# DinoBektesevic/lfd

Measured on AMD Instinct MI355X. Metric: SDSS frames/sec (2048x1489) full detecttrails pipe, higher is better.
Workload: dtype f32

## Files before the change

lfd_amd/csrc/k_hough.h:

```cpp
#pragma once
#include "common.h"
#include "../../include/lfdmi.h"

#define PIXLIST_WORDS 8
#define CHUNK_MAX 64
__device__ __forceinline__ uint32_t chunk_entry(int y, int x0, int len) {
    return ((uint32_t)(len - 1) << 26) | ((uint32_t)y << 13) | (uint32_t)x0;
}

__global__ void __launch_bounds__(256)
k_pixlist(const u64 *bits0, const u64 *bits1, uint32_t *list0, uint32_t *list1, int *counters, int cm_a, int cm_b, int h, int w,
          size_t list_cap, int *accum_clear, int acc_n, size_t acc_stride, const int *active, int need_detect) {
    int g = blockIdx.y, im = blockIdx.z;
    const u64 *bits = im ? bits1 : bits0;
    uint32_t *list = im ? list1 : list0;
    const int cidx = im ? C_NPIX_BOX : C_NPIX_EQU, cidx_b = im ? C_NPIXB_BOX : C_NPIXB_EQU, nnz_idx = im ? C_NNZ_BOX : C_NNZ_EQU;
    if (accum_clear) accum_clear += (size_t)im * acc_stride;
    if (slot_off(active, counters, g)) return;
    int *cnt = counters + g * C_COUNT;
    if (need_detect && !cnt[C_DETECT]) return;
    int wq = LFD_WQ(w);
    if (accum_clear)
        for (int k = blockIdx.x * 256 + threadIdx.x; k < acc_n; k += gridDim.x * 256) accum_clear[(size_t)g * 2 * acc_stride + k] = 0;
    const int nw = h * wq;
// ... 328 lines not shown
            u64 v = pg[k];
            if (v < prev && v > best) best = v;
        }
        for (int off = 32; off > 0; off >>= 1) {
            u64 o = __shfl_down(best, off);
            if (o > best) best = o;
        }
        if (lfd_lane() == 0) red[threadIdx.x >> 6] = best;
        __syncthreads();
        if (threadIdx.x == 0) {
            u64 b = red[0];
            for (int k = 1; k < 4; k++) if (red[k] > b) b = red[k];
            prev_s = b;
            float ro = 0.f, th = 0.f;
            if (b) key_to_line(b, numrho, rho, theta, &ro, &th);
            lg[2 * round] = ro;
            lg[2 * round + 1] = th;
        }
        __syncthreads();
        prev = prev_s;
        if (!prev) {
            if (threadIdx.x == 0)
                for (int r2 = round + 1; r2 < K; r2++) { lg[2 * r2] = 0.f; lg[2 * r2 + 1] = 0.f; }
            break;
        }
    }
}

__global__ void __launch_bounds__(1024)
k_hough_sort(u64 *peaks, const int *counters, float *lines, int max_lines, int numrho, float rho,
             float theta, size_t peak_cap) {
    int g = blockIdx.y, im = blockIdx.x;
    const int *cnt = counters + g * C_COUNT;
    if (cnt[C_OVERFLOW]) return;
    u64 *pg = peaks + ((size_t)g * 2 + im) * peak_cap;
    int n = cnt[im ? C_NPEAK_BOX : C_NPEAK_EQU];
    if ((size_t)n > peak_cap) n = (int)peak_cap;
    int np2 = 1;
    while (np2 < n) np2 <<= 1;
    for (int k = n + threadIdx.x; k < np2; k += 1024) pg[k] = 0;
    __syncthreads();
    for (int size = 2; size <= np2; size <<= 1)
        for (int stride = size >> 1; stride > 0; stride >>= 1) {
            for (int t = threadIdx.x; t < (np2 >> 1); t += 1024) {
                int lo = 2 * t - (t & (stride - 1));
                int hi = lo + stride;
                bool desc = ((lo & size) == 0);
                u64 a = pg[lo], b = pg[hi];
                if (desc ? (a < b) : (a > b)) { pg[lo] = b; pg[hi] = a; }
            }
            __syncthreads();
        }
    int m = min(n, max_lines);
    float *lg = lines + (size_t)g * max_lines * 2;
    for (int k = threadIdx.x; k < m; k += 1024) key_to_line(pg[k], numrho, rho, theta, &lg[2 * k], &lg[2 * k + 1]);
}

__device__ double np_pairwise_dev(const double *a, int n) {
    if (n < 8) {
        double res = 0.;
        for (int i = 0; i < n; i++) res = __dadd_rn(res, a[i]);
        return res;
    }
    double r[8], res;
    int i;
    for (int j = 0; j < 8; j++) r[j] = a[j];
    for (i = 8; i < n - (n % 8); i += 8)
        for (int j = 0; j < 8; j++) r[j] = __dadd_rn(r[j], a[i + j]);
    res = __dadd_rn(__dadd_rn(__dadd_rn(r[0], r[1]), __dadd_rn(r[2], r[3])),
                    __dadd_rn(__dadd_rn(r[4], r[5]), __dadd_rn(r[6], r[7])));
    for (; i < n; i++) res = __dadd_rn(res, a[i]);
    return res;
}
__device__ double np_mean_dev(const double *a, int n) {
    return __ddiv_rn(__dadd_rn(a[0], np_pairwise_dev(a + 1, n - 1)), (double)n);
}

struct TailParams {
    int navg;
    double dro, thetaTresh, lineSetTresh;
    int which;
};

__global__ void k_finalize(const float *lines, const int *counters, lfdmi_result *res, int *need_dim,
                           int *pass_flags, const int *active, TailParams tp, int G) {
    int g = blockIdx.x * blockDim.x + threadIdx.x;
    if (g >= G) return;
    if (active && !active[g]) { if (need_dim) need_dim[g] = 0; return; }
    const int *cnt = counters + g * C_COUNT;
    lfdmi_result r = res[g];
    r.detection = cnt[C_DETECT];
    r.rejected_by_theta = 0;
    r.n_lines_equ = r.n_lines_box = 0;
    if (cnt[C_OVERFLOW]) {
        r.status = LFDMI_ERR_CAPACITY;
        r.x1 = max(cnt[C_NRUNF], cnt[C_NRUNB]);
        r.y1 = cnt[C_NKEYS];
        r.x2 = cnt[C_NSLOTS];
        r.y2 = max(max(cnt[C_NPIX_EQU], cnt[C_NPIX_BOX]), max(cnt[C_NPIXB_EQU], cnt[C_NPIXB_BOX]));
        r.n_lines_equ = max(cnt[C_NPEAK_EQU], cnt[C_NPEAK_BOX]);
    }
    if (r.detection && r.status == 0) {
        int n1 = cnt[C_NPEAK_EQU], n2 = cnt[C_NPEAK_BOX];
        r.n_lines_equ = n1; r.n_lines_box = n2;
        if (n1 == 0 || n2 == 0) {
            r.status = LFDMI_ERR_NOLINES;
        } else {
            int K = tp.navg;
            const float *l1 = lines + ((size_t)g * 2 + 0) * K * 2, *l2 = lines + ((size_t)g * 2 + 1) * K * 2;
            double ro1[LFDMI_MAX_SET_LINES], ro2[LFDMI_MAX_SET_LINES], t1[LFDMI_MAX_SET_LINES],
                t2[LFDMI_MAX_SET_LINES];
            for (int i = 0; i < K; i++) {
                ro1[i] = ro2[i] = t1[i] = t2[i] = 0.;
                if (i >= n1) continue;
                ro1[i] = l1[2 * i];
                if (i >= n2) continue;
                ro2[i] = l2[2 * i];
                t1[i] = l1[2 * i + 1];
                t2[i] = l2[2 * i + 1];
            }
            bool rej = fabs(__dsub_rn(np_mean_dev(ro1, K), np_mean_dev(ro2, K))) > tp.dro;
            if (!rej) {
                double mx = t1[0], mn = t1[0];
                for (int i = 1; i < K; i++) { mx = fmax(mx, t1[i]); mn = fmin(mn, t1[i]); }
                rej = fabs(__dsub_rn(mx, mn)) > tp.thetaTresh;
            }
            if (!rej) {
                double mx = t2[0], mn = t2[0];
                for (int i = 1; i < K; i++) { mx = fmax(mx, t2[i]); mn = fmin(mn, t2[i]); }
                rej = fabs(__dsub_rn(mx, mn)) > tp.thetaTresh;
            }
            if (!rej) {
                for (int i = 0; i < K; i++) ro1[i] = fabs(__dsub_rn(t1[i], t2[i]));
                rej = np_mean_dev(ro1, K) > tp.lineSetTresh;
            }
            if (rej) r.rejected_by_theta = 1;
            else { r.found = tp.which; r.rho = l1[0]; r.theta = l1[1]; }
        }
    }
    res[g] = r;
    pass_flags[g] |= (tp.which == 1) ? (r.detection ? 1 : 0) : (2 | (r.detection ? 4 : 0));
    if (need_dim) need_dim[g] = (r.found == 0 && r.status == 0) ? 1 : 0;
}

__global__ void k_hough_reset(int *counters, int G) {
    int g = blockIdx.x * blockDim.x + threadIdx.x;
    if (g >= G) return;
    int *cnt = counters + g * C_COUNT;
    cnt[C_NPIX_EQU] = 0; cnt[C_NPIX_BOX] = 0; cnt[C_NPIXB_EQU] = 0; cnt[C_NPIXB_BOX] = 0; cnt[C_NPEAK_EQU] = 0; cnt[C_NPEAK_BOX] = 0;
    cnt[C_NNZ_EQU] = 0; cnt[C_NNZ_BOX] = 0;
}

__global__ void k_init_results(lfdmi_result *res, int *pass_flags, int G) {
    int g = blockIdx.x * blockDim.x + threadIdx.x;
    if (g >= G) return;
    pass_flags[g] = 0;
    lfdmi_result r;
    r.status = 0; r.found = 0; r.rho = 0.f; r.theta = 0.f;
    r.x1 = r.y1 = r.x2 = r.y2 = 0;
    r.n_lines_equ = r.n_lines_box = 0; r.detection = 0; r.rejected_by_theta = 0;
    res[g] = r;
}
```

lfd_amd/csrc/k_image.h:

```cpp
#pragma once
#include <type_traits>
#include "common.h"
#include "../../include/lfdmi.h"

struct RsDev {
    int defaultxy, maxxy, magcount, filter_index;
    double pixscale, maxmagdiff, filter_cap;
};

__device__ __forceinline__ void py_slice(long start, long stop, long len, int *a, int *b) {
    if (start < 0) { start += len; if (start < 0) start = 0; } else if (start > len) start = len;
    if (stop < 0) { stop += len; if (stop < 0) stop = 0; } else if (stop > len) stop = len;
    *a = (int)start; *b = (int)stop;
}

__global__ void __launch_bounds__(256)
k_rs_boxes(int h, int w, int max_obj, const int *count, const float *rowc, const float *colc, const float *psfmag,
           const float *petro90, const int *nobserve, const int *ndetect, RsDev p, int4 *boxes) {
    const int f = blockIdx.y, i = blockIdx.x * 256 + threadIdx.x;
    if (i >= max_obj) return;
    int r0 = 0, r1 = 0, c0 = 0, c1 = 0;
    if (i < count[f]) {
        size_t o5 = ((size_t)f * max_obj + i) * 5, o1 = (size_t)f * max_obj + i;
        int fi = p.filter_index;
        long x = (long)ceil((double)colc[o5 + fi]);
        long y = (long)ceil((double)rowc[o5 + fi]);
        long mags[5];
        for (int k = 0; k < 5; k++) mags[k] = (long)ceil((double)psfmag[o5 + k]);
        bool ok = (double)mags[fi] < p.filter_cap;
        int cnt = 0;
        for (int j = 0; j < 5; j++)
            for (int k = j + 1; k < 5; k++) {
                long d = mags[j] - mags[k];
                if (d < 0) d = -d;
                if ((double)d > p.maxmagdiff) cnt++;
            }
        ok = ok && (p.magcount >= cnt);
        long dxy = p.defaultxy;
        long pet = (long)ceil((double)petro90[o5 + fi]);
        if (pet > 0) dxy = (long)((double)pet / p.pixscale) + 10;
        if (dxy > p.maxxy) dxy = p.defaultxy;
        ok = ok && (nobserve[o1] == ndetect[o1]);
        if (ok) {
            py_slice(x - dxy, x + dxy, h, &r0, &r1);
            py_slice(y - dxy, y + dxy, w, &c0, &c1);
        }
    }
    boxes[(size_t)f * max_obj + i] = make_int4(r0, r1, c0, c1);
}

__global__ void __launch_bounds__(256)
k_rs_fill(float *frames, int h, int w, int max_obj, const int *count, const int4 *boxes, int bx0) {
    int f = blockIdx.y, i = (blockIdx.x + bx0) * 4 + (threadIdx.x >> 6), lane = threadIdx.x & 63;
    if (i >= max_obj) return;
    const int4 bx = boxes[(size_t)f * max_obj + i];
    const int r0 = __builtin_amdgcn_readfirstlane(bx.x), r1 = __builtin_amdgcn_readfirstlane(bx.y);
    const int c0 = __builtin_amdgcn_readfirstlane(bx.z), c1 = __builtin_amdgcn_readfirstlane(bx.w);
    int nc = c1 - c0;
    if (r1 <= r0 || nc <= 0) return;
    float *img = frames + (size_t)f * h * w;
    if (nc <= 32) {
        for (int r = r0 + (lane >> 5); r < r1; r += 2)
            if ((lane & 31) < nc) img[(size_t)r * w + c0 + (lane & 31)] = 0.0f;
    } else {
        for (int r = r0; r < r1; r++)
            for (int c = c0 + lane; c < c1; c += 64) img[(size_t)r * w + c] = 0.0f;
    }
}

#define RS_SORT_MIN 1024
#define RS_SORT_MAXH 8192
__global__ void __launch_bounds__(1024)
k_rs_sort(int h, int max_obj, const int *count, const int4 *boxes, int4 *sboxes, int *rowstart) {
    const int f = blockIdx.x, n = min(count[f], max_obj);
    __shared__ int cur[RS_SORT_MAXH + 1];
    __shared__ int wsum[16];
    const int4 *bx = boxes + (size_t)f * max_obj;
    for (int r = threadIdx.x; r <= h; r += 1024) cur[r] = 0;
    __syncthreads();
    for (int i = threadIdx.x; i < n; i += 1024) {
        const int4 b = bx[i];
        if (b.y > b.x && b.w > b.z) atomicAdd(&cur[b.x], 1);
    }
    __syncthreads();
    const int per = (h + 1 + 1023) / 1024, r0 = threadIdx.x * per, lane = threadIdx.x & 63, wv = threadIdx.x >> 6;
    int loc = 0;
    for (int k = 0; k < per; k++) if (r0 + k <= h) loc += cur[r0 + k];
    int inc = loc;
    for (int off = 1; off < 64; off <<= 1) { int t = __shfl_up(inc, off); if (lane >= off) inc += t; }
    if (lane == 63) wsum[wv] = inc;
    __syncthreads();
    int base = inc - loc;
    for (int k = 0; k < wv; k++) base += wsum[k];
    for (int k = 0; k < per; k++)
        if (r0 + k <= h) {
            const int c = cur[r0 + k];
            cur[r0 + k] = base;
            rowstart[(size_t)f * (h + 1) + r0 + k] = base;
            base += c;
        }
    __syncthreads();
    for (int i = threadIdx.x; i < n; i += 1024) {
// ... 486 lines not shown
    }
    const uint8_t *gs = gsrc + (size_t)g * N;
    const u64 *db = dbits + (size_t)g * nw;
    __shared__ unsigned short qlist[4][512];
    __shared__ int qyq[4][64];
    const int wvi = threadIdx.x >> 6;
    qyq[wvi][lane] = (y << 8) | q;
    u64 rem = e;
    for (;;) {
        const int cnt = min(__popcll(rem), 8);
        int incl = cnt;
        for (int off = 1; off < 64; off <<= 1) {
            int t = __shfl_up(incl, off);
            if (lane >= off) incl += t;
        }
        const int total = __shfl(incl, 63);
        if (total == 0) break;
        int o = incl - cnt;
        for (int k = 0; k < cnt; k++) {
            const int bb = __ffsll((long long)rem) - 1;
            rem &= rem - 1;
            qlist[wvi][o++] = (unsigned short)((lane << 6) | bb);
        }
        __builtin_amdgcn_wave_barrier();
        for (int t = lane; t < total; t += 64) {
            const unsigned ent = qlist[wvi][t];
            const int yq = qyq[wvi][ent >> 6];
            const int yy0 = yq >> 8, x = ((yq & 0xff) << 6) + (int)(ent & 63u);
            auto val = [&](int yy, int xx) -> unsigned {
                if (yy < 0 || yy >= h || xx < 0 || xx >= w) return 255u;
                return (unsigned)gs[(size_t)yy * w + xx] + (unsigned)((db[(size_t)yy * wq + (xx >> 6)] >> (xx & 63)) & 1ull);
            };
            unsigned m = 255u;
            if (kh == 3 && kw == 3 && x >= 1 && x + 2 < w && yy0 >= 1 && yy0 + 1 < h) {
                unsigned gv[3];
                u64 bw0[3], bw1[3];
                const int xb = x - 1, wi = xb >> 6, sh = xb & 63;
#pragma unroll
                for (int k = 0; k < 3; k++) {
                    const size_t ro = (size_t)(yy0 + k - 1);
                    uint32_t t4;
                    __builtin_memcpy(&t4, gs + ro * w + xb, 4);
                    gv[k] = t4;
                    bw0[k] = db[ro * wq + wi];
                    bw1[k] = sh > 61 ? db[ro * wq + wi + 1] : 0ull;
                }
#pragma unroll
                for (int k = 0; k < 3; k++) {
                    const unsigned bits = (unsigned)((bw0[k] >> sh) | (sh > 61 ? bw1[k] << (64 - sh) : 0ull)) & 7u;
                    m = min(m, (gv[k] & 0xffu) + (bits & 1u));
                    m = min(m, ((gv[k] >> 8) & 0xffu) + ((bits >> 1) & 1u));
                    m = min(m, ((gv[k] >> 16) & 0xffu) + ((bits >> 2) & 1u));
                }
            } else if (kh == 3 && kw == 3) {
                unsigned v9[9];
#pragma unroll
                for (int k = 0; k < 9; k++) v9[k] = val(yy0 + k / 3 - 1, x + k % 3 - 1);
#pragma unroll
                for (int k = 0; k < 9; k++) m = min(m, v9[k]);
            } else {
                for (int dy = 0; dy < kh; dy++)
                    for (int dx = 0; dx < kw; dx++) m = min(m, val(yy0 + dy - ay, x + dx - ax));
            }
            d[(size_t)yy0 * w + x] = (uint8_t)m;
        }
        __builtin_amdgcn_wave_barrier();
    }
    }
}

__global__ void __launch_bounds__(256)
k_hist_u8(const uint8_t *src, size_t N, int *hist) {
    int g = blockIdx.y;
    __shared__ int sh[256];
    sh[threadIdx.x] = 0;
    __syncthreads();
    const uint8_t *s = src + (size_t)g * N;
    for (size_t k = (size_t)blockIdx.x * 256 + threadIdx.x; k < N; k += (size_t)gridDim.x * 256)
        atomicAdd(&sh[s[k]], 1);
    __syncthreads();
    if (sh[threadIdx.x]) atomicAdd(&hist[g * 256 + threadIdx.x], sh[threadIdx.x]);
}

__global__ void __launch_bounds__(256)
k_lut(const int *hist, int total, uint8_t *lut, const int *active) {
    int g = blockIdx.x, t = threadIdx.x;
    if (active && !active[g]) return;
    __shared__ int cum[256];
    __shared__ int first;
    int hv = hist[g * 256 + t];
    cum[t] = hv;
    if (t == 0) first = 256;
    __syncthreads();
    if (hv) atomicMin(&first, t);
    for (int off = 1; off < 256; off <<= 1) {
        int v = (t >= off) ? cum[t - off] : 0;
        __syncthreads();
        cum[t] += v;
        __syncthreads();
    }
    int f = first;
    if (f >= 256) { lut[g * 256 + t] = 0; return; }
    int hf = hist[g * 256 + f];
    unsigned out;
    if (hf == total) out = (unsigned)f;
    else if (t <= f) out = 0;
    else {
        float scale = __fdiv_rn(255.f, (float)(total - hf));
        out = sat_u8_f32(__fmul_rn((float)(cum[t] - cum[f]), scale));
    }
    lut[g * 256 + t] = (uint8_t)out;
}

__global__ void __launch_bounds__(256)
k_apply_lut(const uint8_t *src, const uint8_t *lut, uint8_t *dst, size_t N) {
    int g = blockIdx.y;
    __shared__ uint8_t l[256];
    l[threadIdx.x] = lut[g * 256 + threadIdx.x];
    __syncthreads();
    for (size_t k = (size_t)blockIdx.x * 256 + threadIdx.x; k < N; k += (size_t)gridDim.x * 256)
        dst[(size_t)g * N + k] = l[src[(size_t)g * N + k]];
}

typedef unsigned short dcw_us2 __attribute__((ext_vector_type(2)));
__device__ __forceinline__ uint32_t dcw_pkmax(uint32_t a, uint32_t b) {
    return __builtin_bit_cast(uint32_t, __builtin_elementwise_max(__builtin_bit_cast(dcw_us2, a), __builtin_bit_cast(dcw_us2, b)));
}
__device__ __forceinline__ uint32_t dcw_pkmin(uint32_t a, uint32_t b) {
    return __builtin_bit_cast(uint32_t, __builtin_elementwise_min(__builtin_bit_cast(dcw_us2, a), __builtin_bit_cast(dcw_us2, b)));
}
template <int S, int NWT, bool MIN = false>
__device__ __forceinline__ void dcw_shift_max(uint32_t (&E)[NWT], uint32_t (&O)[NWT], int nw) {
    constexpr int K = S / 4, R = S % 4;
#pragma unroll
    for (int i = 0; i < NWT; i++) {
        if (i >= nw || i + K + 1 >= NWT) continue;
        uint32_t e2, o2;
        if constexpr (R == 0) { e2 = E[i + K]; o2 = O[i + K]; }
        else if constexpr (R == 1) { e2 = O[i + K]; o2 = __builtin_amdgcn_alignbyte(E[i + K + 1], E[i + K], 2); }
        else if constexpr (R == 2) { e2 = __builtin_amdgcn_alignbyte(E[i + K + 1], E[i + K], 2); o2 = __builtin_amdgcn_alignbyte(O[i + K + 1], O[i + K], 2); }
        else { e2 = __builtin_amdgcn_alignbyte(O[i + K + 1], O[i + K], 2); o2 = E[i + K + 1]; }
        E[i] = MIN ? dcw_pkmin(E[i], e2) : dcw_pkmax(E[i], e2);
        O[i] = MIN ? dcw_pkmin(O[i], o2) : dcw_pkmax(O[i], o2);
    }
}
template <int KW, bool MIN = false, int BASE = 12>
__device__ __forceinline__ uint32_t dcw_hmax(const uint32_t *rw, int jj) {
    constexpr int AX = KW / 2, R0 = (BASE - AX) & 3, Q0 = (BASE - AX) >> 2;
    constexpr int NB = KW + 3, NW = (NB + 3) / 4, NR = (R0 + NB + 3) / 4, NWT = NW + 9;
    uint32_t raw[NR + 1];
#pragma unroll
    for (int i = 0; i < NR; i++) raw[i] = rw[Q0 + jj + i];
    raw[NR] = 0;
    uint32_t E[NWT], O[NWT];
#pragma unroll
    for (int i = 0; i < NWT; i++) {
        uint32_t a = 0;
        if (i < NW) a = R0 ? __builtin_amdgcn_alignbyte(raw[i + 1 <= NR ? i + 1 : NR], raw[i], R0) : raw[i];
        E[i] = a & 0x00FF00FFu;
        O[i] = (a >> 8) & 0x00FF00FFu;
    }
    constexpr int P = KW >= 16 ? 16 : (KW >= 8 ? 8 : (KW >= 4 ? 4 : (KW >= 2 ? 2 : 1))), D = KW - P;
    constexpr int need1 = 4 + D + (P > 8 ? 8 : 0) + (P > 4 ? 4 : 0) + (P > 2 ? 2 : 0);
    if constexpr (P >= 2) dcw_shift_max<1, NWT, MIN>(E, O, (need1 + 3) / 4);
    constexpr int need2 = need1 - 2;
    if constexpr (P >= 4) dcw_shift_max<2, NWT, MIN>(E, O, (need2 + 3) / 4);
    constexpr int need4 = need2 - 4;
    if constexpr (P >= 8) dcw_shift_max<4, NWT, MIN>(E, O, (need4 + 3) / 4);
    if constexpr (P >= 16) dcw_shift_max<8, NWT, MIN>(E, O, (4 + D + 3) / 4);
    if constexpr (D > 0) dcw_shift_max<D, NWT, MIN>(E, O, 1);
    return E[0] | (O[0] << 8);
}

#define MORPH_TW 64
#define MORPH_TH 32

template <int OP>
__global__ void __launch_bounds__(256)
k_morph_rect(const uint8_t *src, uint8_t *dst, u64 *bits, const uint8_t *lut, int h, int w, int kh,
             int kw, const int *active) {
    int g = blockIdx.z;
    if (active && !active[g]) return;
    extern __shared__ uint8_t sm[];
    const int IH = MORPH_TH + kh - 1, IW = MORPH_TW + kw - 1;
    uint8_t *tin = sm;
    uint8_t *tmp = sm + ((IH * IW + 15) & ~15);
    __shared__ uint8_t slut[256];
    const int fill = OP ? 255 : 0;
    int x0 = blockIdx.x * MORPH_TW, y0 = blockIdx.y * MORPH_TH;
    int ay = kh / 2, ax = kw / 2;
    size_t N = (size_t)h * w;
    const uint8_t *s = src + (size_t)g * N;
    if (lut) slut[threadIdx.x] = lut[g * 256 + threadIdx.x];
    for (int idx = threadIdx.x; idx < IH * IW; idx += 256) {
// ... 1095 lines not shown
```

lfd_amd/csrc/lfdmi.hip:

```cpp
#include <hip/hip_runtime.h>

#include <math.h>
#include <stdio.h>
#include <stdlib.h>
#include <time.h>
#include <pthread.h>
#include <sched.h>
#include <string.h>

#include <atomic>
#include <condition_variable>
#include <string>
#include <thread>
#include <mutex>
#include <memory>
#include <vector>

#include "../../include/lfdmi.h"
#include "common.h"
#include "k_ccl.h"
#include "k_hough.h"
#include "k_image.h"
#include "k_rect.h"
#include "k_frame.h"
// ... 20 lines not shown
struct TimedSpan { hipEvent_t a, b; int group, pass, det; };

struct CallChunk {
    int c0, nc;
    bool general_on, scan_fused;
    long long growths;
};
struct PendingCall {
    int kind = 0;
    int status = 0;
    bool finished = false;
    void *frames = nullptr;
    size_t frame_bytes = 0;
    int dtype = 0, n = 0, h = 0, w = 0, loc = 0;
    bool host_blot = false;
    lfdmi_catalog cat{};
    bool has_cat = false, has_rs = false;
    lfdmi_rs_params rs{};
    lfdmi_params p1{}, p2{};
    std::vector<uint8_t> kern;
    int flip = 0, dim = 0, prep_mode = 0, n_scales = 1;
    double rhos[LFDMI_MAX_SCALES] = {0};
    lfdmi_result *results = nullptr;
    std::vector<CallChunk> chunks;
    void *pin = nullptr;
    size_t pin_bytes = 0;
    int *flags_h = nullptr;
    lfdmi_result *rec_h = nullptr;
    int4 *boxes_h = nullptr;
    hipEvent_t done = nullptr;
};

struct lfdmi_ctx {
    int device = 0, H = 0, W = 0, G = 0, wq = 0;
    size_t N = 0;
    hipStream_t stream = nullptr;
    bool own_stream = true;
    hipStream_t side[2] = {nullptr, nullptr};
    hipEvent_t ev_fork = nullptr, ev_join[2] = {nullptr, nullptr};
    std::string err;
    uint8_t *gray = nullptr, *tmp = nullptr, *equ = nullptr, *lut = nullptr, *mask = nullptr;
    int *hist = nullptr;
    u64 *candb = nullptr, *strongb = nullptr, *edgeb = nullptr, *equb = nullptr, *boxb = nullptr;
    int *Lf = nullptr, *YMf = nullptr, *FLf = nullptr, *Lb = nullptr, *YMb = nullptr, *FLb = nullptr;
    int *SBf = nullptr, *SBb = nullptr, *PAb = nullptr, *ROWf = nullptr, *ROWb = nullptr;
    int *scanf_ = nullptr, *scanb_ = nullptr;
    int run_cap = 0;
    int4 *keys = nullptr;
    int *bigkeys = nullptr, *medkeys = nullptr;
    int *wl_fg = nullptr, *wl_bg = nullptr;
    int2 *rowext = nullptr;
    int *quads = nullptr;
    uint32_t *pix_equ = nullptr, *pix_box = nullptr;
    int *accum = nullptr;
    u64 *peaks = nullptr;
    float *lines = nullptr, *tab = nullptr;
    int *counters = nullptr, *need_dim = nullptr;
    uint8_t *zero_block = nullptr;
    size_t zero_bytes = 0, zero_counters_off = 0;
    uint8_t *zero_block2 = nullptr;
    size_t zero_bytes2 = 0;
    u64 *cellbm2 = nullptr;
    u64 *candmask = nullptr;
    u64 *fullbits = nullptr;
    int *hist2 = nullptr;
    bool fuse_dual = false;
    u64 *dbits = nullptr, *nzd = nullptr;
    bool sparse_erode_fill = true;
    bool delta_dim = true;
    int delta_state = 0;
    int dual_state = 0;
    int2 *rsa = nullptr;
    long long *prof = nullptr;
    u64 *cellbm = nullptr;
    int bm_bands = 0;
    bool use_cellbm = true;
    int4 *segcnt = nullptr;
    int *fg_keys = nullptr;
    bool fg_keys_on = true;
    int *fb_fg = nullptr, *fb_bg = nullptr;
    int *perm = nullptr;
    const int *perm_cur = nullptr;
    bool use_perm = true;
    int *perm_tiles = nullptr;
    bool use_tile_perm = true;
    bool sky_fast = true;
    bool vote_classes = true;
    bool rs_fold_on = true;
    bool rs_fold = false;
    const int *rs_count_dev = nullptr; int rs_max_obj = 0;
    int rs_fill_at = 13;
    int rs_fill_at0 = 3, rs_fill_part = 0;
    float *rs_fill_frames = nullptr;
    int rs_fill_nc = 0, rs_fill_h = 0, rs_fill_w = 0;
    hipEvent_t ev_rsfill = nullptr;
    bool rs_fill_inflight = false;
    bool scan_fused = true;
    u64 *scan_partial = nullptr;
    int scan_epoch = 0;
    int scan_spin = 4096;
    bool rects_prep = true;
    bool vote_balance = true;
    lfdmi_result *res_dev = nullptr;
    void *res_host = nullptr;
    bool worst = false;
    lfdmi_ctx *spill = nullptr;
    long long n_spilled = 0;
    long long n_scan_giveups = 0, n_general_reruns = 0, n_general_chunks = 0, n_chunks = 0, n_cap_growths = 0;
    bool grow_on = true;
    bool scan_fused_cfg = true;
    int scan_quiet = 0, scan_rearm = 64;
    size_t bytes = 0;
    double min_rho = 1.0;
    void *scratch = nullptr;
    size_t scratch_bytes = 0;
    int last_h = 0, last_w = 0;
    int quiet_chunks = 0;
    void *feed_pin[2] = {nullptr, nullptr}, *feed_dev[2] = {nullptr, nullptr};
    size_t feed_bytes = 0, feed_pin_bytes = 0;
    bool feed_cpus_known = false;
    hipStream_t feed_copy = nullptr, feed_copy2 = nullptr;
    hipEvent_t feed_mid = nullptr;
    int feed_streams = 2;
    hipEvent_t feed_up[2] = {nullptr, nullptr};
    int feed_threads = 4;
    size_t feed_chunk_bytes = 800u << 20;
    std::vector<int> feed_cpus;
    int fail_chunk = -1;
    int4 *rs_sboxes = nullptr;
    int *rs_rowstart = nullptr;
    size_t rs_rowstart_cap = 0;
    bool rs_sorted = false;
    int rs_sort_min = RS_SORT_MIN;
    int rs_hmax = 0;
    int4 *rs_boxes = nullptr;
    size_t rs_boxes_cap = 0;
    void *stage = nullptr;
    size_t stage_bytes = 0;
    void *cat_dev = nullptr;
    size_t cat_bytes = 0;
    int key_cap = 0, slot_cap = 0;
    size_t acc_cap = 0, peak_cap = 0, list_cap = 0, peak_worst = 0;
    struct HoughTab {
        double rho = -1, theta = -1;
        int h = 0, w = 0, numangle = 0, numrho = 0;
        long long stamp = 0;
        std::vector<float> host;
    } tabs[LFDMI_MAX_SCALES];
    long long tab_clock = 0;
    int tab_cur = 0;
    int numangle = 0, numrho = 0;
    bool timing = false;
    uint64_t timing_mask = 0;
    std::vector<TimedSpan> spans;
    std::vector<hipEvent_t> ev_pool;
    float t_ms[TG_COUNT] = {0};
    int t_n[TG_COUNT] = {0};
    long long t_units[TG_COUNT] = {0};
    int stage_mode = -1;
    bool stages_valid = false;
    bool eroded_valid = false;
    int vote_split = 4;
    int vote_aw = -1;
    int pe_rows = 12;
    bool fuse_prep_erode = true;
    bool general_seen = false, general_on = true;
// ... 118 lines not shown
static void worst_caps(int h, int w, lfdmi_caps *c) {
    size_t N = (size_t)h * w;
    c->run_cap = (int)((size_t)h * (w / 2 + 1) + 16);
    c->key_cap = (int)(N / 2 + 16);
    c->slot_cap = (int)(2 * N + 4 * (size_t)h + 16);
    c->list_cap = (int)N;
    c->peak_cap = 0;
    c->min_rho = 1.0;
}

extern "C" void lfdmi_default_caps(int max_h, int max_w, lfdmi_caps *out) {
    size_t N = (size_t)max_h * max_w;
    lfdmi_caps wc;
    worst_caps(max_h, max_w, &wc);
    auto pick = [](size_t want, size_t floor_, int worst) { size_t v = want > floor_ ? want : floor_; return (int)(v < (size_t)worst ? v : (size_t)worst); };
    out->run_cap = pick(N / 16, 16384, wc.run_cap);
    out->key_cap = pick(N / 256, 4096, wc.key_cap);
    out->slot_cap = pick(N / 16, 16384, wc.slot_cap);
    out->list_cap = pick(N / 16, 16384, wc.list_cap);
    out->peak_cap = 65536;
    out->min_rho = 5.0;
}

static int create_impl(int device, int max_h, int max_w, int max_inflight, const lfdmi_caps *caps_in, lfdmi_ctx **out) {
    if (!out || max_h <= 0 || max_w <= 0 || max_inflight <= 0 || max_h > 8191 || max_w > 8191) return LFDMI_ERR_ARG;
    lfdmi_ctx *ctx = new lfdmi_ctx();
    *out = ctx;
    ctx->device = device; ctx->H = max_h; ctx->W = max_w; ctx->G = max_inflight;
    if (const char *e = getenv("LFDMI_FRAME_CCL")) ctx->frame_ccl = atoi(e) != 0;
    if (const char *e = getenv("LFDMI_FUSE_PREP_ERODE")) ctx->fuse_prep_erode = atoi(e) != 0;
    if (const char *e = getenv("LFDMI_FUSE_DUAL")) ctx->fuse_dual = atoi(e) != 0;
    if (const char *e = getenv("LFDMI_DELTA_DIM")) ctx->delta_dim = atoi(e) != 0;
    if (const char *e = getenv("LFDMI_SPARSE_ERODE_FILL")) ctx->sparse_erode_fill = atoi(e) != 0;
    if (const char *e = getenv("LFDMI_VOTE_SPLIT")) { int v = atoi(e); if (v >= 1 && v <= 16) ctx->vote_split = v; }
    if (const char *e = getenv("LFDMI_VOTE_AW")) { int v = atoi(e); if (*e && v >= 0 && v <= 6) ctx->vote_aw = v; }
    if (const char *e = getenv("LFDMI_PE_ROWS")) { int v = atoi(e); if (v >= 2 && v <= 64) ctx->pe_rows = v; }
    if (const char *e = getenv("LFDMI_FRAME_DBG")) ctx->frame_dbg = atoi(e);
    if (const char *e = getenv("LFDMI_FRAME_RUNCAP")) { int v = atoi(e); if (v >= 0 && v < FRAME_RUNCAP) ctx->frame_runcap = v; }
    if (const char *e = getenv("LFDMI_FRAME_LDS")) {
        int v = atoi(e);
        if (v >= 32 && v <= FRAME_RUNCAP) { ctx->frame_lds = (v + 31) & ~31; ctx->frame_runcap = std::min(ctx->frame_runcap, ctx->frame_lds); }
    }
    if (const char *e = getenv("LFDMI_DC_SUBSTRIPS")) { int v = atoi(e); if (v >= 1 && v <= 64) ctx->dc_substrips = v; }
    if (const char *e = getenv("LFDMI_DC_STRIP")) { int v = atoi(e); if (v >= 1 && v <= DCW_MAXS) ctx->dc_strip = v; }
    if (const char *e = getenv("LFDMI_DC_TILELIST")) ctx->dc_tilelist = atoi(e) != 0;
    if (const char *e = getenv("LFDMI_DC_PARTS")) { int v = atoi(e); if (v >= 1 && v <= 4096) ctx->dc_parts = v; }
    if (const char *e = getenv("LFDMI_FEED_STREAMS")) { int v = atoi(e); if (v == 1 || v == 2) ctx->feed_streams = v; }
    if (const char *e = getenv("LFDMI_FEED_THREADS")) { int v = atoi(e); if (v >= 1 && v <= 64) ctx->feed_threads = v; }
    if (const char *e = getenv("LFDMI_FEED_MB")) { int v = atoi(e); if (v >= 0 && v <= 8192) ctx->feed_chunk_bytes = (size_t)v << 20; }
    ctx->N = (size_t)max_h * max_w;
    ctx->wq = LFD_WQ(max_w);
    size_t N = ctx->N, G = (size_t)max_inflight, BW = (size_t)max_h * ctx->wq;
    lfdmi_caps wc, caps;
    worst_caps(max_h, max_w, &wc);
    if (caps_in) caps = *caps_in; else lfdmi_default_caps(max_h, max_w, &caps);
    if (const char *e = getenv("LFDMI_WORST_CASE")) if (atoi(e)) caps = wc;
    auto cap = [](int v, int worst) { return (v <= 0 || v > worst) ? worst : v; };
    ctx->run_cap = cap(caps.run_cap, wc.run_cap);
    ctx->key_cap = cap(caps.key_cap, wc.key_cap);
    ctx->slot_cap = cap(caps.slot_cap, wc.slot_cap);
    ctx->list_cap = (size_t)cap(caps.list_cap, wc.list_cap);
    ctx->min_rho = caps.min_rho >= 1.0 ? caps.min_rho : 1.0;
    int na, nr;
    lfdmi_hough_dims(max_h, max_w, ctx->min_rho, LFD_PI / 180, &na, &nr);
    ctx->acc_cap = (size_t)(na + 2) * (nr + 2);
    size_t peak_worst = next_pow2((size_t)na * nr);
    ctx->peak_cap = caps.peak_cap > 0 ? next_pow2((size_t)caps.peak_cap) : peak_worst;
    if (ctx->peak_cap > peak_worst) ctx->peak_cap = peak_worst;
    ctx->peak_worst = peak_worst;
    ctx->worst = ctx->run_cap == wc.run_cap && ctx->key_cap == wc.key_cap && ctx->slot_cap == wc.slot_cap &&
                 ctx->list_cap == (size_t)wc.list_cap && ctx->peak_cap == peak_worst && ctx->min_rho <= 1.0;
    HIPCHK(hipSetDevice(device));
    HIPCHK(hipStreamCreateWithFlags(&ctx->stream, hipStreamNonBlocking));
    for (int i = 0; i < 2; i++) {
        HIPCHK(hipStreamCreateWithFlags(&ctx->side[i], hipStreamNonBlocking));
        HIPCHK(hipEventCreateWithFlags(&ctx->ev_join[i], hipEventDisableTiming));
    }
    HIPCHK(hipEventCreateWithFlags(&ctx->ev_fork, hipEventDisableTiming));
    HIPCHK(hipEventCreateWithFlags(&ctx->ev_rsfill, hipEventDisableTiming));
    RET(dmalloc(ctx, &ctx->gray, G * N));
    RET(dmalloc(ctx, &ctx->tmp, G * N));
    RET(dmalloc(ctx, &ctx->equ, G * N));
    RET(dmalloc(ctx, &ctx->lut, G * 256));
    RET(dmalloc(ctx, &ctx->mask, (size_t)LFDMI_MAX_MORPH_K * LFDMI_MAX_MORPH_K * 2));
    RET(dmalloc(ctx, &ctx->candb, G * BW));
    RET(dmalloc(ctx, &ctx->strongb, G * BW));
    RET(dmalloc(ctx, &ctx->edgeb, G * BW));
    RET(dmalloc(ctx, &ctx->equb, G * BW));
    RET(dmalloc(ctx, &ctx->boxb, G * BW));
    RET(dmalloc(ctx, &ctx->dbits, G * BW));
    RET(dmalloc(ctx, &ctx->nzd, G * BW));
    for (int **p : {&ctx->Lf, &ctx->YMf, &ctx->FLf, &ctx->Lb, &ctx->YMb, &ctx->FLb, &ctx->SBf, &ctx->SBb, &ctx->PAb,
                    &ctx->ROWf, &ctx->ROWb})
        RET(dmalloc(ctx, p, G * ctx->run_cap));
    if (const char *e = getenv("LFDMI_DC_PROFILE")) ctx->dc_profile = atoi(e) != 0;
    if (const char *e = getenv("LFDMI_DC_SPECIALIZE")) ctx->dc_specialize = atoi(e) != 0;
    if (getenv("LFDMI_FRAME_PROFILE") || ctx->dc_profile) RET(dmalloc(ctx, &ctx->prof, G * 16));
    RET(dmalloc(ctx, &ctx->rsa, G * FRAME_RUNCAP));
    ctx->bm_bands = (max_h + CELLBM_ROWS - 1) / CELLBM_ROWS;
    if (const char *e = getenv("LFDMI_CELLBM")) ctx->use_cellbm = atoi(e) != 0;
    ctx->tile_cap = ((max_h + DCW_TH - 1) / DCW_TH) * ((max_w + CANNY_TW - 1) / CANNY_TW);
    RET(dmalloc(ctx, &ctx->tile_list, G * ctx->tile_cap));
    RET(dmalloc(ctx, &ctx->segcnt, G * SCAN_MAX_SEG));
    RET(dmalloc(ctx, &ctx->perm, G));
    RET(dmalloc(ctx, &ctx->perm_tiles, G));
    if (const char *e = getenv("LFDMI_TILE_PERM")) ctx->use_tile_perm = atoi(e) != 0;
    if (const char *e = getenv("LFDMI_SKY_FAST")) ctx->sky_fast = atoi(e) != 0;
    if (const char *e = getenv("LFDMI_VOTE_CLASSES")) ctx->vote_classes = atoi(e) != 0;
    if (const char *e = getenv("LFDMI_VOTE_BALANCE")) ctx->vote_balance = atoi(e) != 0;
    if (const char *e = getenv("LFDMI_RECTS_PREP")) ctx->rects_prep = atoi(e) != 0;
    if (const char *e = getenv("LFDMI_RS_FOLD")) ctx->rs_fold_on = atoi(e) != 0;
    if (const char *e = getenv("LFDMI_RS_SORT_MIN")) ctx->rs_sort_min = atoi(e);
    if (const char *e = getenv("LFDMI_SCAN_FUSED")) ctx->scan_fused = atoi(e) != 0;
    ctx->scan_fused_cfg = ctx->scan_fused;
    if (const char *e = getenv("LFDMI_GROW")) ctx->grow_on = atoi(e) != 0;
    if (const char *e = getenv("LFDMI_SCAN_REARM")) ctx->scan_rearm = std::max(1, atoi(e));
    if (const char *e = getenv("LFDMI_SCAN_SPIN")) ctx->scan_spin = std::max(0, atoi(e));
    if (const char *e = getenv("LFDMI_SCAN_EPOCH0")) ctx->scan_epoch = atoi(e) & ((1 << 22) - 1);
    if (const char *e = getenv("LFDMI_RS_FILL_AT")) ctx->rs_fill_at = atoi(e);
    if (const char *e = getenv("LFDMI_RS_FILL_AT0")) ctx->rs_fill_at0 = atoi(e);
    if (const char *e = getenv("LFDMI_PERM")) ctx->use_perm = atoi(e) != 0;
    RET(dmalloc(ctx, &ctx->fb_fg, G));
    RET(dmalloc(ctx, &ctx->fg_keys, G));
    HIPCHK(hipMemsetAsync(ctx->fg_keys, 0, G * sizeof(int), ctx->stream));
    if (const char *e = getenv("LFDMI_FG_KEYS")) ctx->fg_keys_on = atoi(e) != 0;
    RET(dmalloc(ctx, &ctx->fb_bg, G));
    RET(dmalloc(ctx, &ctx->scanf_, G * BW));
    RET(dmalloc(ctx, &ctx->scanb_, G * BW));
    RET(dmalloc(ctx, &ctx->keys, G * ctx->key_cap));
    RET(dmalloc(ctx, &ctx->bigkeys, G * ctx->key_cap));
    RET(dmalloc(ctx, &ctx->medkeys, G * ctx->key_cap));
    RET(dmalloc(ctx, &ctx->wl_fg, G * BW));
    RET(dmalloc(ctx, &ctx->wl_bg, G * BW));
    RET(dmalloc(ctx, &ctx->rowext, G * ctx->slot_cap));
    RET(dmalloc(ctx, &ctx->quads, G * ctx->key_cap * 8));
    RET(dmalloc(ctx, &ctx->pix_equ, G * 2 * ctx->list_cap));
    RET(dmalloc(ctx, &ctx->pix_box, G * 2 * ctx->list_cap));
    RET(dmalloc(ctx, &ctx->accum, G * 2 * ctx->acc_cap));
    RET(dmalloc(ctx, &ctx->peaks, G * 2 * ctx->peak_cap));
    RET(dmalloc(ctx, &ctx->lines, G * 2 * LFDMI_MAX_SET_LINES * 2));
    RET(dmalloc(ctx, &ctx->tab, (size_t)LFDMI_MAX_SCALES * 2 * MAX_ANGLES));
    {
        size_t nb_cnt = G * C_COUNT * sizeof(int), nb_hist = G * 256 * sizeof(int), nb_bm = G * ctx->bm_bands * CELLBM_WORDS * sizeof(u64);
        uint8_t *blk = nullptr;
        RET(dmalloc(ctx, &blk, nb_bm + nb_hist + nb_cnt));
        ctx->cellbm = (u64 *)blk;
        ctx->hist = (int *)(blk + nb_bm);
        ctx->counters = (int *)(blk + nb_bm + nb_hist);
        ctx->zero_block = blk;
        ctx->zero_bytes = nb_bm + nb_hist + nb_cnt;
        ctx->zero_counters_off = nb_bm + nb_hist;
        uint8_t *blk2 = nullptr;
        RET(dmalloc(ctx, &blk2, nb_bm + nb_hist));
        ctx->cellbm2 = (u64 *)blk2;
        ctx->hist2 = (int *)(blk2 + nb_bm);
        ctx->zero_block2 = blk2;
        ctx->zero_bytes2 = nb_bm + nb_hist;
        RET(dmalloc(ctx, &ctx->fullbits, G * (size_t)max_h * ((max_w + 255) >> 8)));
        RET(dmalloc(ctx, &ctx->candmask, G * (size_t)((max_h + MORPH_TH - 1) / MORPH_TH) * 2));
    }
    RET(dmalloc(ctx, &ctx->need_dim, G));
    RET(dmalloc(ctx, &ctx->scan_partial, G * SCAN_MAX_BLK));
    HIPCHK(hipMemsetAsync(ctx->scan_partial, 0, G * SCAN_MAX_BLK * sizeof(u64), ctx->stream));
    {
        char *blk = nullptr;
        RET(dmalloc(ctx, &blk, G * sizeof(int) + G * LFDMI_MAX_SCALES * sizeof(lfdmi_result)));
        ctx->pass_flags = (int *)blk;
        ctx->res_dev = (lfdmi_result *)(blk + G * sizeof(int));
        HIPCHK(hipHostMalloc(&ctx->res_host, G * sizeof(int) + G * sizeof(lfdmi_result), hipHostMallocDefault));
    }
    HIPCHK(hipFuncSetAttribute((const void *)k_hough_vote<6>, hipFuncAttributeMaxDynamicSharedMemorySize, 160 * 1024 - 64));
    HIPCHK(hipFuncSetAttribute((const void *)k_hough_vote<5>, hipFuncAttributeMaxDynamicSharedMemorySize, 160 * 1024 - 64));
    HIPCHK(hipFuncSetAttribute((const void *)k_hough_vote<4>, hipFuncAttributeMaxDynamicSharedMemorySize, 160 * 1024 - 64));
    HIPCHK(hipFuncSetAttribute((const void *)k_hough_vote<3>, hipFuncAttributeMaxDynamicSharedMemorySize, 160 * 1024 - 64));
    HIPCHK(hipFuncSetAttribute((const void *)k_hough_vote<2>, hipFuncAttributeMaxDynamicSharedMemorySize, 160 * 1024 - 64));
    HIPCHK(hipFuncSetAttribute((const void *)k_hough_vote<1>, hipFuncAttributeMaxDynamicSharedMemorySize, 160 * 1024 - 64));
    HIPCHK(hipFuncSetAttribute((const void *)k_hough_vote<0>, hipFuncAttributeMaxDynamicSharedMemorySize, 160 * 1024 - 64));
    HIPCHK(hipFuncSetAttribute((const void *)k_rects_big, hipFuncAttributeMaxDynamicSharedMemorySize, 160 * 1024 - 64));
    HIPCHK(hipFuncSetAttribute((const void *)k_dilate_canny_v, hipFuncAttributeMaxDynamicSharedMemorySize, 64 * 1024));
    HIPCHK(hipFuncSetAttribute((const void *)k_frame_fg, hipFuncAttributeMaxDynamicSharedMemorySize, 160 * 1024 - 1024));
    HIPCHK(hipFuncSetAttribute((const void *)k_prep_erode<false, 0>, hipFuncAttributeMaxDynamicSharedMemorySize, 140 * 1024));
    HIPCHK(hipFuncSetAttribute((const void *)k_prep_erode<false, 1>, hipFuncAttributeMaxDynamicSharedMemorySize, 140 * 1024));
    HIPCHK(hipFuncSetAttribute((const void *)k_prep_erode<false, 2>, hipFuncAttributeMaxDynamicSharedMemorySize, 140 * 1024));
    HIPCHK(hipFuncSetAttribute((const void *)k_prep_erode<false, 3>, hipFuncAttributeMaxDynamicSharedMemorySize, 140 * 1024));
    HIPCHK(hipFuncSetAttribute((const void *)k_prep_erode<true, LFDMI_PREP_BRIGHT_THEN_DIM>, hipFuncAttributeMaxDynamicSharedMemorySize, 140 * 1024));
    HIPCHK(hipFuncSetAttribute((const void *)k_frame_contours, hipFuncAttributeMaxDynamicSharedMemorySize,
                               (FRAME_RUNCAP + 4 * (FRAME_RUNCAP / 32)) * (int)sizeof(int)));
    HIPCHK(hipFuncSetAttribute((const void *)k_morph_rect<0>, hipFuncAttributeMaxDynamicSharedMemorySize, 64 * 1024));
    HIPCHK(hipFuncSetAttribute((const void *)k_morph_rect<1>, hipFuncAttributeMaxDynamicSharedMemorySize, 64 * 1024));
    return 0;
}

extern "C" int lfdmi_ctx_create(int device, int max_h, int max_w, int max_inflight, lfdmi_ctx **out) {
    return create_impl(device, max_h, max_w, max_inflight, nullptr, out);
}
extern "C" int lfdmi_ctx_create_sized(int device, int max_h, int max_w, int max_inflight, const lfdmi_caps *caps, lfdmi_ctx **out) {
    return create_impl(device, max_h, max_w, max_inflight, caps, out);
}
extern "C" int64_t lfdmi_ctx_bytes(lfdmi_ctx *ctx) {
    return ctx ? (int64_t)(ctx->bytes + ctx->trail.bytes + (ctx->spill ? ctx->spill->bytes : 0)) : 0;
}
extern "C" int64_t lfdmi_spill_count(lfdmi_ctx *ctx) { return ctx ? ctx->n_spilled : 0; }
extern "C" int lfdmi_get_stats(lfdmi_ctx *ctx, int64_t *out, int n) {
    if (!ctx || !out || n < 0 || n > LFDMI_STAT_COUNT) return LFDMI_ERR_ARG;
// ... 254 lines not shown
    }
    return 0;
}

static int rs_fill_point(lfdmi_ctx *ctx, int k) {
    if (!ctx->rs_fill_frames) return 0;
    const bool first = k >= 0 && k == ctx->rs_fill_at0 && ctx->rs_fill_part == 0 && !ctx->rs_sorted;
    const bool rest = k < 0 || k == ctx->rs_fill_at;
    if (!first && !rest) return 0;
    float *fr = ctx->rs_fill_frames;
    static const int side_i = getenv("LFDMI_RS_FILL_SIDE") ? (atoi(getenv("LFDMI_RS_FILL_SIDE")) & 1) : 1;
    hipStream_t sd = ctx->side[side_i];
    HIPCHK(hipEventRecord(ctx->ev_rsfill, ctx->stream));
    HIPCHK(hipStreamWaitEvent(sd, ctx->ev_rsfill, 0));
    {
        Span sp(ctx, KID_REMOVESTARS, 0, sd);
        if (ctx->rs_sorted)
            k_rs_fill_bands<<<dim3((ctx->rs_fill_h + RS_BAND_ROWS - 1) / RS_BAND_ROWS, ctx->rs_fill_nc), 256, 0, sd>>>(
                fr, ctx->rs_fill_h, ctx->rs_fill_w, ctx->rs_max_obj, ctx->rs_sboxes, ctx->rs_rowstart, ctx->rs_hmax);
        else {
            static const double frac = getenv("LFDMI_RS_FILL_FRAC") ? atof(getenv("LFDMI_RS_FILL_FRAC")) : 0.5;
            const int nblk = (ctx->rs_max_obj + 3) / 4, half = std::max(0, std::min(nblk, (int)(nblk * frac)));
            const int b0 = ctx->rs_fill_part ? half : 0, b1 = first ? half : nblk;
            if (b1 > b0)
                k_rs_fill<<<dim3(b1 - b0, ctx->rs_fill_nc), 256, 0, sd>>>(fr, ctx->rs_fill_h, ctx->rs_fill_w, ctx->rs_max_obj,
                                                                          ctx->rs_count_dev, ctx->rs_boxes, b0);
        }
        KCHK("k_rs_fill");
    }
    HIPCHK(hipEventRecord(ctx->ev_rsfill, sd));
    ctx->rs_fill_inflight = true;
    if (first) ctx->rs_fill_part = 1;
    else { ctx->rs_fill_frames = nullptr; ctx->rs_fill_part = 0; }
    return 0;
}

static dim3 word_grid(int h, int w, int n) { return dim3((unsigned)((h * LFD_WQ(w) + 255) / 256), (unsigned)n); }

static int run_prep(lfdmi_ctx *ctx, const void *src, int dtype, int nc, int h, int w, int flip, int mode,
                    double minFlux, double addFlux, const int *active, bool zeroed = false, u64 *fullbits = nullptr,
                    const lfdmi_params *delta_dim = nullptr) {
    if (!zeroed) {
        HIPCHK(hipMemsetAsync(ctx->hist, 0, (size_t)nc * 256 * sizeof(int), ctx->stream));
        HIPCHK(hipMemsetAsync(ctx->cellbm, 0, (size_t)nc * ctx->bm_bands * CELLBM_WORDS * sizeof(u64), ctx->stream));
    }
    {
        Span sp(ctx, KID_PREP_HIST);
        static const int prep_rows = [] {
            const char *e = getenv("LFDMI_PREP_ROWS");
            int v = e ? atoi(e) : 8;
            return (v == 1 || v == 2 || v == 4 || v == 8 || v == 16) ? v : 8;
        }();
        const dim3 pgrid((h + prep_rows - 1) / prep_rows, nc);
#define LFD_PREP_LAUNCH(M_)                                                                                                          \
    k_prep_hist<M_><<<pgrid, 256, 0, ctx->stream>>>(src, dtype, h, w, flip, mode, minFlux, addFlux, ctx->gray, ctx->hist, ctx->cellbm, \
                                                    ctx->bm_bands, active, fullbits, prep_rows)
        if (delta_dim) {
#define LFD_PREP_DELTA(P_, RS_)                                                                                                       \
    k_prep_hist<1, true, P_, RS_><<<pgrid, 256, 0, ctx->stream>>>(src, dtype, h, w, flip, mode, minFlux, addFlux, ctx->gray, ctx->hist, \
                                                              ctx->cellbm, ctx->bm_bands, active, fullbits, prep_rows, ctx->dbits,    \
                                                              ctx->hist2, (float)delta_dim->minFlux, (float)delta_dim->addFlux, ctx->nzd, sky_fast, \
                                                              ctx->rs_sorted ? ctx->rs_sboxes : ctx->rs_boxes, ctx->rs_count_dev, ctx->rs_max_obj, \
                                                              ctx->rs_sorted ? ctx->rs_rowstart : nullptr, ctx->rs_hmax)
            const bool sky_on = ctx->sky_fast;
            const float mfa = (float)delta_dim->minFlux + (float)delta_dim->addFlux;
            const int sky_fast = (sky_on && mode == LFDMI_PREP_BRIGHT && mfa > 0.5f) ? 1 : 0;
            const bool rs = ctx->rs_fold && w <= RS_MAXW && prep_rows <= RS_MAXROWS;
            if ((float)delta_dim->minFlux > 0.f) { if (rs) LFD_PREP_DELTA(true, true); else LFD_PREP_DELTA(true, false); }
            else { if (rs) LFD_PREP_DELTA(false, true); else LFD_PREP_DELTA(false, false); }
#undef LFD_PREP_DELTA
        } else
        if (dtype == LFDMI_F32 && (w & 3) == 0) {
            switch (mode & 3) {
            case 0: LFD_PREP_LAUNCH(0); break;
            case 1: LFD_PREP_LAUNCH(1); break;
            case 2: LFD_PREP_LAUNCH(2); break;
            default: LFD_PREP_LAUNCH(3); break;
            }
        } else LFD_PREP_LAUNCH(-1);
#undef LFD_PREP_LAUNCH
        KCHK("k_prep_hist");
    }
    Span sp(ctx, KID_LUT);
    k_lut<<<nc, 256, 0, ctx->stream>>>(ctx->hist, h * w, ctx->lut, active);
    KCHK("k_lut");
    return 0;
}

static bool all_ones(const uint8_t *k, int kh, int kw) {
    for (int i = 0; i < kh * kw; i++) if (!k[i]) return false;
    return true;
}

static int run_morph(lfdmi_ctx *ctx, const uint8_t *src, uint8_t *dst, u64 *bits, const uint8_t *lut, const uint8_t *kernel,
                     int kh, int kw, int op, int nc, int h, int w, const int *active, const u64 *fullbits = nullptr, u64 *cellout = nullptr,
                     bool *marked = nullptr, bool sparse_fill = false) {
    if (marked) *marked = false;
    if (!kernel || kh <= 0 || kw <= 0 || kh > LFDMI_MAX_MORPH_K || kw > LFDMI_MAX_MORPH_K)
        return fail(ctx, LFDMI_ERR_UNSUPPORTED, "structuring element must be 1..31 on both sides");
    Span sp(ctx, op ? KID_ERODE : KID_DILATE);
    if (all_ones(kernel, kh, kw) && (w % 16) == 0) {
        int IH = MORPH_TH + kh - 1;
        size_t lds = (size_t)IH * (MORPH_TW + 2 * MORPH_HALO) + (size_t)IH * MORPH_TW * 2 + (size_t)MORPH_TH * MORPH_TW;
        dim3 grid((w + MORPH_TW - 1) / MORPH_TW, (h + MORPH_TH - 1) / MORPH_TH, nc);
        const u64 *cand = nullptr;
        if (op == 1 && fullbits && kw >= 7 && !lut && !bits && grid.x <= 128 && kh <= 33) {
            sparse_fill = sparse_fill && cellout && kh <= 9 && kw <= 33;
            k_erode_cand<<<dim3(grid.y, nc), 64, 0, ctx->stream>>>(fullbits, ctx->candmask, dst, h, w, kh, active, sparse_fill ? 0 : 1);
            KCHK("k_erode_cand");
            cand = ctx->candmask;
        }
        if (op == 0) k_morph_rect_v<0><<<grid, 256, lds, ctx->stream>>>(src, dst, bits, lut, h, w, kh, kw, active, cellout, ctx->bm_bands);
        else if (cand) {
            dim3 rgrid(grid.y, nc);
            if (kh == 9 && kw == 9 && ctx->dc_specialize)
                k_morph_rect_rows<1, 9, 9><<<rgrid, 256, lds, ctx->stream>>>(src, dst, lut, h, w, kh, kw, active, cand, cellout, ctx->bm_bands);
            else k_morph_rect_rows<1><<<rgrid, 256, lds, ctx->stream>>>(src, dst, lut, h, w, kh, kw, active, cand, cellout, ctx->bm_bands);
        } else if (kh == 9 && kw == 9 && ctx->dc_specialize)
            k_morph_rect_v<1, 9, 9><<<grid, 256, lds, ctx->stream>>>(src, dst, bits, lut, h, w, kh, kw, active, cellout, ctx->bm_bands);
        else k_morph_rect_v<1><<<grid, 256, lds, ctx->stream>>>(src, dst, bits, lut, h, w, kh, kw, active, cellout, ctx->bm_bands);
        if (marked) *marked = cellout != nullptr;
        KCHK("k_morph_rect_v");
        if (cand && sparse_fill) {
            k_fill_around<<<dim3(grid.y, nc), 64, 0, ctx->stream>>>(cand, cellout, ctx->bm_bands, dst, h, w, active);
            KCHK("k_fill_around");
        }
    } else if (all_ones(kernel, kh, kw)) {
        int IH = MORPH_TH + kh - 1, IW = MORPH_TW + kw - 1;
        size_t lds = ((size_t)(IH * IW + 15) & ~(size_t)15) + (size_t)IH * MORPH_TW;
        dim3 grid((w + MORPH_TW - 1) / MORPH_TW, (h + MORPH_TH - 1) / MORPH_TH, nc);
        if (op == 0) k_morph_rect<0><<<grid, 256, lds, ctx->stream>>>(src, dst, bits, lut, h, w, kh, kw, active);
        else k_morph_rect<1><<<grid, 256, lds, ctx->stream>>>(src, dst, bits, lut, h, w, kh, kw, active);
        KCHK("k_morph_rect");
    } else {
        uint8_t *m = ctx->mask + (op ? LFDMI_MAX_MORPH_K * LFDMI_MAX_MORPH_K : 0);
        HIPCHK(hipMemcpyAsync(m, kernel, (size_t)kh * kw, hipMemcpyHostToDevice, ctx->stream));
        dim3 grid((w + 63) / 64, (h + 3) / 4, nc);
        if (op == 0) k_morph_generic<0><<<grid, 256, 0, ctx->stream>>>(src, dst, bits, lut, m, h, w, kh, kw, active);
        else k_morph_generic<1><<<grid, 256, 0, ctx->stream>>>(src, dst, bits, lut, m, h, w, kh, kw, active);
        KCHK("k_morph_generic");
    }
    return 0;
}

static int run_scan(lfdmi_ctx *ctx, const u64 *bits, int val, int *scan, int cidx, int nc, int h, int w, int *wl_fg, int *wl_bg,
                    u64 *clear, const int *active) {
    int nseg = (h * LFD_WQ(w) + 63) / 64;
    dim3 grid((nseg + SCANW_WAVES * SCAN_SEGS - 1) / (SCANW_WAVES * SCAN_SEGS), nc);
    if (ctx->scan_fused && (int)grid.x <= SCAN_MAX_BLK) {
        if (++ctx->scan_epoch >= (1 << 22)) {
            HIPCHK(hipMemsetAsync(ctx->scan_partial, 0, (size_t)ctx->G * SCAN_MAX_BLK * sizeof(u64), ctx->stream));
            ctx->scan_epoch = 1;
        }
        k_scan_fused<<<grid, 64 * SCANW_WAVES, 0, ctx->stream>>>(bits, val, ctx->scan_partial, ctx->scan_epoch, ctx->scan_spin, ctx->pass_flags, scan, h, w, wl_fg, wl_bg, clear,
                                                                  ctx->counters, cidx, ctx->run_cap, active);
        KCHK("k_scan_fused");
        return 0;
    }
    k_scan_count<<<grid, 64 * SCANW_WAVES, 0, ctx->stream>>>(bits, val, ctx->segcnt, h, w, wl_fg != nullptr, active);
    KCHK("k_scan_count");
    k_scan_bases<<<nc, SCAN_THREADS, 0, ctx->stream>>>(ctx->segcnt, ctx->counters, cidx, h, w, ctx->run_cap, wl_fg != nullptr, active);
    KCHK("k_scan_bases");
    k_scan_write<<<grid, 64 * SCANW_WAVES, 0, ctx->stream>>>(bits, val, ctx->segcnt, scan, h, w, wl_fg, wl_bg, clear, active);
    KCHK("k_scan_write");
    return 0;
}
// ... 421 lines not shown
                                                                   ctx->acc_cap, active, need_detect, rng, balance); \
        break;
        switch (aw_log2) {
            LFD_LAUNCH_VOTE(6) LFD_LAUNCH_VOTE(5) LFD_LAUNCH_VOTE(4) LFD_LAUNCH_VOTE(3) LFD_LAUNCH_VOTE(2)
            LFD_LAUNCH_VOTE(1) LFD_LAUNCH_VOTE(0)
        }
#undef LFD_LAUNCH_VOTE
        KCHK("k_hough_vote");
    }
    { Span sp(ctx, KID_PEAKS, need_detect);
    static const int peak_rows = getenv("LFDMI_PEAK_ROWS") ? std::max(8, atoi(getenv("LFDMI_PEAK_ROWS"))) : 32;
    k_hough_peaks<<<dim3(std::min(32, std::max(1, nr / peak_rows)), n_img, nc), std::min(256, (na + 63) / 64 * 64), 0, ctx->stream>>>(ctx->accum, ctx->peaks, ctx->counters, na, nr, threshold,
                                                                ctx->acc_cap, ctx->peak_cap, active, need_detect);
    KCHK("k_hough_peaks"); }
    if (K > 0) {
        Span sp(ctx, KID_TOPK, need_detect);
        k_hough_topk<<<dim3(n_img, nc), 256, 0, ctx->stream>>>(ctx->peaks, ctx->counters, ctx->lines, K, nr, (float)rho, (float)theta,
                                                               ctx->peak_cap, active, need_detect);
        KCHK("k_hough_topk");
    }
    return 0;
}

static int check_params(lfdmi_ctx *ctx, const lfdmi_params *p, bool dim) {
    if (!p) return fail(ctx, LFDMI_ERR_ARG, "params NULL");
    if (p->gaussKernel < 0 || p->gaussKernel > 31 || (p->gaussKernel > 0 && (p->gaussKernel & 1) == 0))
        return fail(ctx, LFDMI_ERR_ARG, "gaussKernel must be 0 (off) or odd, 1..31");
    if (p->nlinesInSet < 1 || p->nlinesInSet > LFDMI_MAX_SET_LINES) return fail(ctx, LFDMI_ERR_ARG, "nlinesInSet out of range");
    if (!p->dilateKernel) return fail(ctx, LFDMI_ERR_ARG, "dilateKernel NULL");
    if (dim && !p->erodeKernel) return fail(ctx, LFDMI_ERR_ARG, "erodeKernel NULL");
    return 0;
}

static int prep_erode_rows(const lfdmi_ctx *ctx, int w, int kh) {
    int BR = ctx->pe_rows;
    while (BR > 2 && (size_t)(2 * BR + kh - 1) * (w + 32) > 60 * 1024) BR >>= 1;
    if ((size_t)(2 * BR + kh - 1) * (w + 32) + 16 > 140 * 1024) return 0;
    return BR >= 2 * (kh - 1) ? BR : 0;
}

static bool can_fuse_prep_erode(const lfdmi_ctx *ctx, int dtype, int w, const uint8_t *kernel, int kh, int kw) {
    if (!ctx->fuse_prep_erode || ctx->keep_equ || dtype != LFDMI_F32 || (w % 16) != 0) return false;
    if (!kernel || kh <= 0 || kw <= 0 || kh > LFDMI_MAX_MORPH_K || kw > LFDMI_MAX_MORPH_K || !all_ones(kernel, kh, kw)) return false;
    return kw / 2 <= 16 && kw - 1 - kw / 2 <= 16 && prep_erode_rows(ctx, w, kh) > 0;
}

static int run_prep_erode(lfdmi_ctx *ctx, const void *src, int nc, int h, int w, int flip, int mode, double minFlux, double addFlux,
                          int kh, int kw, const int *active, bool from_bits = false) {
    int BR = prep_erode_rows(ctx, w, kh);
    size_t lds = (size_t)(2 * BR + kh - 1) * (w + 32) + 16;
    if (from_bits) {
        Span sp(ctx, KID_BITS_ERODE);
        const int nwords = h * LFD_WQ(w);
        k_bits_erode<<<dim3((nwords + 256 * BE_REP - 1) / (256 * BE_REP), nc), 256, 0, ctx->stream>>>(ctx->gray, ctx->dbits, ctx->nzd, ctx->tmp, ctx->cellbm2,
                                                                             ctx->bm_bands, h, w, kh, kw, active);
        KCHK("k_bits_erode");
        return 0;
    }
    {
        Span sp(ctx, KID_PREP_ERODE);
#define LFD_PE_LAUNCH(M_)                                                                                                             \
    k_prep_erode<false, M_><<<dim3((h + BR - 1) / BR, nc), PE_THREADS, lds, ctx->stream>>>(                                           \
        (const float *)src, h, w, flip, mode, (float)minFlux, (float)addFlux, ctx->tmp, ctx->hist, kh, kw, BR, ctx->cellbm, ctx->bm_bands, \
        active, nullptr, nullptr, nullptr)
        switch (mode & 3) {
        case 0: LFD_PE_LAUNCH(0); break;
        case 1: LFD_PE_LAUNCH(1); break;
        case 2: LFD_PE_LAUNCH(2); break;
        default: LFD_PE_LAUNCH(3); break;
        }
#undef LFD_PE_LAUNCH
        KCHK("k_prep_erode");
    }
    Span sp(ctx, KID_LUT);
    k_lut<<<nc, 256, 0, ctx->stream>>>(ctx->hist, h * w, ctx->lut, active);
    KCHK("k_lut");
    return 0;
}

static int run_prep_dual(lfdmi_ctx *ctx, const void *src, int nc, int h, int w, int flip, const lfdmi_params *dimp) {
    int kh = dimp->erode_kh, kw = dimp->erode_kw;
    int BR = prep_erode_rows(ctx, w, kh);
    size_t lds = (size_t)(2 * BR + kh - 1) * (w + 32) + 16;
    HIPCHK(hipMemsetAsync(ctx->zero_block2, 0, ctx->zero_bytes2, ctx->stream));
    {
        Span sp(ctx, KID_PREP_DUAL);
        k_prep_erode<true, LFDMI_PREP_BRIGHT_THEN_DIM><<<dim3((h + BR - 1) / BR, nc), PE_THREADS, lds, ctx->stream>>>((const float *)src, h, w, flip, LFDMI_PREP_BRIGHT_THEN_DIM,
                                                                              (float)dimp->minFlux, (float)dimp->addFlux, ctx->tmp, ctx->hist2, kh, kw, BR,
                                                                              ctx->cellbm2, ctx->bm_bands, nullptr, ctx->gray, ctx->hist, ctx->cellbm);
        KCHK("k_prep_dual");
    }
    Span sp(ctx, KID_LUT);
    k_lut<<<nc, 256, 0, ctx->stream>>>(ctx->hist, h * w, ctx->lut, nullptr);
    KCHK("k_lut");
    return 0;
}

static int run_front(lfdmi_ctx *ctx, const void *src, int dtype, int nc, int h, int w, int flip, int prep_mode, bool dim,
                     const lfdmi_params *p, const int *active, const lfdmi_params *dual_dim = nullptr) {
    const uint8_t *dil_src = ctx->gray;
    const u64 *bm = ctx->cellbm;
    ctx->eroded_valid = dim;
    ctx->perm_cur = nullptr;
    if (active && ctx->use_perm) {
        k_active_perm<<<1, 64, 0, ctx->stream>>>(active, nc, ctx->perm);
        KCHK("k_active_perm");
        ctx->perm_cur = ctx->perm;
    }
    if (dim && ctx->delta_state == 2) {
        HIPCHK(hipMemsetAsync(ctx->zero_block + ctx->zero_counters_off, 0, ctx->zero_bytes - ctx->zero_counters_off, ctx->stream));
        HIPCHK(hipMemsetAsync(ctx->cellbm2, 0, (size_t)nc * ctx->bm_bands * CELLBM_WORDS * sizeof(u64), ctx->stream));
        { Span sp(ctx, KID_LUT);
          k_lut<<<nc, 256, 0, ctx->stream>>>(ctx->hist2, h * w, ctx->lut, active);
          KCHK("k_lut"); }
        RET(run_prep_erode(ctx, nullptr, nc, h, w, 0, 0, 0, 0, p->erode_kh, p->erode_kw, active, true));
        dil_src = ctx->tmp;
        bm = ctx->cellbm2;
    } else
    if (dim && ctx->dual_state == 2) {
        HIPCHK(hipMemsetAsync(ctx->zero_block + ctx->zero_counters_off, 0, ctx->zero_bytes - ctx->zero_counters_off, ctx->stream));
        Span sp(ctx, KID_LUT);
        k_lut<<<nc, 256, 0, ctx->stream>>>(ctx->hist2, h * w, ctx->lut, active);
        KCHK("k_lut");
        dil_src = ctx->tmp;
        bm = ctx->cellbm2;
    } else {
    HIPCHK(hipMemsetAsync(ctx->zero_block, 0, ctx->zero_bytes, ctx->stream));
    if (!dim && dual_dim && ctx->delta_state != 1) {
        RET(run_prep_dual(ctx, src, nc, h, w, flip, dual_dim));
    } else
    if (dim && can_fuse_prep_erode(ctx, dtype, w, p->erodeKernel, p->erode_kh, p->erode_kw)) {
        RET(run_prep_erode(ctx, src, nc, h, w, flip, prep_mode, p->minFlux, p->addFlux, p->erode_kh, p->erode_kw, active));
        dil_src = ctx->tmp;
    } else {
        const bool wide = dim && p->erode_kw >= 7 && dtype == LFDMI_F32 && (w & 3) == 0 && p->erode_kh <= 33;
        if (dim) HIPCHK(hipMemsetAsync(ctx->zero_block2, 0, ctx->zero_bytes2, ctx->stream));
        const lfdmi_params *dd = (!dim && ctx->delta_state == 1) ? dual_dim : nullptr;
        if (dd) HIPCHK(hipMemsetAsync(ctx->hist2, 0, (size_t)nc * 256 * sizeof(int), ctx->stream));
        RET(run_prep(ctx, src, dtype, nc, h, w, flip, prep_mode, p->minFlux, p->addFlux, active, true, wide ? ctx->fullbits : nullptr, dd));
        RET(rs_fill_point(ctx, 1));
        if (dim) {
            bool marked = false;
            const bool only_tiles = wide && !ctx->keep_equ && ctx->sparse_erode_fill && p->gaussKernel <= 0 && ctx->use_cellbm && ctx->dc_tilelist &&
                                    p->dilate_kh <= 9 && p->dilate_kh <= DCW_MAXKH && can_fuse_dilate_canny(p->dilateKernel, p->dilate_kh, p->dilate_kw, w) &&
                                    (w + CANNY_TW - 1) / CANNY_TW <= 128 && (h + DCW_TH - 1) / DCW_TH <= DCT_MAXBANDS;
            RET(run_morph(ctx, ctx->gray, ctx->tmp, nullptr, nullptr, p->erodeKernel, p->erode_kh, p->erode_kw, 1, nc, h, w, active,
                          wide ? ctx->fullbits : nullptr, ctx->cellbm2, &marked, only_tiles));
            if (only_tiles) ctx->eroded_valid = false;
            dil_src = ctx->tmp;
            if (marked) bm = ctx->cellbm2;
        }
    }
    }
    if (p->gaussKernel > 0) {
        RET(run_morph(ctx, dil_src, ctx->equ, ctx->equb, ctx->lut, p->dilateKernel, p->dilate_kh, p->dilate_kw, 0, nc, h, w, active));
        RET(ensure_scratch(ctx, (size_t)ctx->G * ctx->N));
        RET(run_gauss(ctx, ctx->equ, (uint8_t *)ctx->scratch, nc, h, w, p->gaussKernel, p->gaussSigma, active));
        RET(run_canny(ctx, (const uint8_t *)ctx->scratch, nc, h, w, 0, 255, active, false, true));
    } else if (can_fuse_dilate_canny(p->dilateKernel, p->dilate_kh, p->dilate_kw, w)) {
        RET(run_dilate_canny(ctx, dil_src, nc, h, w, ctx->lut, p->dilate_kh, p->dilate_kw, active, ctx->use_cellbm ? bm : nullptr));
        RET(rs_fill_point(ctx, 2 + 10 * ctx->cur_pass));
        RET(run_canny(ctx, ctx->equ, nc, h, w, 0, 255, active, true, true));
    } else {
        RET(run_morph(ctx, dil_src, ctx->equ, ctx->equb, ctx->lut, p->dilateKernel, p->dilate_kh, p->dilate_kw, 0, nc, h, w, active));
        RET(run_canny(ctx, ctx->equ, nc, h, w, 0, 255, active, false, true));
    }
    return run_rects(ctx, nc, h, w, p->contoursMode, p->contoursMethod, p->minAreaRectMinLen, p->lwTresh, active);
}

static int run_tail(lfdmi_ctx *ctx, int nc, int h, int w, double rho, bool dim, const lfdmi_params *p, const int *active,
                    int *need_dim, lfdmi_result *res, bool again) {
    if (again) {
        k_hough_reset<<<(nc + 63) / 64, 64, 0, ctx->stream>>>(ctx->counters, nc);
        KCHK("k_hough_reset");
    }
    RET(run_hough(ctx, nc, h, w, rho, LFD_PI / 180, 1, 2, p->nlinesInSet, 1, active));
    TailParams tp;
    tp.navg = p->nlinesInSet; tp.dro = p->dro; tp.thetaTresh = p->thetaTresh; tp.lineSetTresh = p->lineSetTresh;
    tp.which = dim ? 2 : 1;
    Span sp(ctx, KID_FINALIZE);
    k_finalize<<<(nc + 63) / 64, 64, 0, ctx->stream>>>(ctx->lines, ctx->counters, res, need_dim, ctx->pass_flags, active, tp, nc);
    KCHK("k_finalize");
    return 0;
}

static int run_pass(lfdmi_ctx *ctx, const void *src, int dtype, int nc, int h, int w, int flip, int prep_mode, bool dim,
                    const lfdmi_params *p, const int *active, int *need_dim, const lfdmi_params *dual_dim = nullptr) {
    RET(run_front(ctx, src, dtype, nc, h, w, flip, prep_mode, dim, p, active, dual_dim));
    ctx->perm_cur = nullptr;
    return run_tail(ctx, nc, h, w, p->houghMethod, dim, p, active, need_dim, ctx->res_dev, false);
}

static void dictify(int h, int w, lfdmi_result *r) {
    if (!r->found) return;
    float c = cosf(r->theta), s = sinf(r->theta);
    float x0 = c * r->rho, y0 = s * r->rho;
    float L = (float)(h + w);
    r->x1 = (int32_t)(x0 - L * s);
    r->y1 = (int32_t)(y0 + L * c);
    r->x2 = (int32_t)(x0 + L * s);
    r->y2 = (int32_t)(y0 - L * c);
}

extern "C" int lfdmi_prep_u8(lfdmi_ctx *ctx, const void *src, int dtype, int n, int h, int w, int flip, int mode,
                             double minFlux, double addFlux, uint8_t *gray, int32_t *hist, int loc) {
    RET(check_shape(ctx, n, h, w));
    if (!src || dtype < 0 || dtype > 2 || mode < 0 || mode > 3) return fail(ctx, LFDMI_ERR_ARG, "lfdmi_prep_u8: bad argument");
    if (dtype == LFDMI_U8 && (mode & 2)) return fail(ctx, LFDMI_ERR_DTYPE, "dim masking needs a float image (numpy refuses uint8 += float)");
    size_t N = (size_t)h * w, es = dtype_size(dtype);
    for (int c0 = 0; c0 < n; c0 += ctx->G) {
        int nc = n - c0 < ctx->G ? n - c0 : ctx->G;
        const void *d;
        RET(in_ptr(ctx, src, (size_t)c0 * N * es, (size_t)nc * N * es, loc, &d));
        RET(run_prep(ctx, d, dtype, nc, h, w, flip, mode, minFlux, addFlux, nullptr));
        RET(out_copy(ctx, gray, (size_t)c0 * N, ctx->gray, (size_t)nc * N, loc));
        RET(out_copy(ctx, hist, (size_t)c0 * 256 * 4, ctx->hist, (size_t)nc * 256 * 4, loc));
        RET(sync(ctx, nc));
    }
    return 0;
}

extern "C" int lfdmi_equalize_hist(lfdmi_ctx *ctx, const uint8_t *src, int n, int h, int w, uint8_t *dst, int loc) {
    RET(check_shape(ctx, n, h, w));
    if (!src || !dst) return fail(ctx, LFDMI_ERR_ARG, "NULL image");
    size_t N = (size_t)h * w;
    for (int c0 = 0; c0 < n; c0 += ctx->G) {
        int nc = n - c0 < ctx->G ? n - c0 : ctx->G;
        const void *d;
        RET(in_ptr(ctx, src, (size_t)c0 * N, (size_t)nc * N, loc, &d));
        {
            Span sp(ctx, KID_MISC);
            HIPCHK(hipMemsetAsync(ctx->hist, 0, (size_t)nc * 256 * sizeof(int), ctx->stream));
            k_hist_u8<<<dim3(256, nc), 256, 0, ctx->stream>>>((const uint8_t *)d, N, ctx->hist);
            KCHK("k_hist_u8");
            k_lut<<<nc, 256, 0, ctx->stream>>>(ctx->hist, h * w, ctx->lut, nullptr);
            KCHK("k_lut");
            k_apply_lut<<<dim3(512, nc), 256, 0, ctx->stream>>>((const uint8_t *)d, ctx->lut, ctx->equ, N);
            KCHK("k_apply_lut");
        }
        RET(out_copy(ctx, dst, (size_t)c0 * N, ctx->equ, (size_t)nc * N, loc));
        RET(sync(ctx, nc));
    }
    return 0;
}

static int morph_api(lfdmi_ctx *ctx, const uint8_t *src, int n, int h, int w, const uint8_t *kernel, int kh, int kw,
                     uint8_t *dst, int loc, int op) {
    RET(check_shape(ctx, n, h, w));
    if (!src || !dst) return fail(ctx, LFDMI_ERR_ARG, "NULL image");
    size_t N = (size_t)h * w;
    for (int c0 = 0; c0 < n; c0 += ctx->G) {
        int nc = n - c0 < ctx->G ? n - c0 : ctx->G;
        const void *d;
        RET(in_ptr(ctx, src, (size_t)c0 * N, (size_t)nc * N, loc, &d));
        RET(run_morph(ctx, (const uint8_t *)d, ctx->equ, nullptr, nullptr, kernel, kh, kw, op, nc, h, w, nullptr));
        RET(out_copy(ctx, dst, (size_t)c0 * N, ctx->equ, (size_t)nc * N, loc));
        RET(sync(ctx, nc));
    }
    return 0;
}
extern "C" int lfdmi_dilate(lfdmi_ctx *ctx, const uint8_t *src, int n, int h, int w, const uint8_t *kernel, int kh, int kw,
                            uint8_t *dst, int loc) { return morph_api(ctx, src, n, h, w, kernel, kh, kw, dst, loc, 0); }
extern "C" int lfdmi_erode(lfdmi_ctx *ctx, const uint8_t *src, int n, int h, int w, const uint8_t *kernel, int kh, int kw,
                           uint8_t *dst, int loc) { return morph_api(ctx, src, n, h, w, kernel, kh, kw, dst, loc, 1); }

extern "C" int lfdmi_gaussian_blur(lfdmi_ctx *ctx, const uint8_t *src, int n, int h, int w, int ksize, double sigma, uint8_t *dst, int loc) {
    RET(check_shape(ctx, n, h, w));
    if (!src || !dst) return fail(ctx, LFDMI_ERR_ARG, "NULL image");
    size_t N = (size_t)h * w;
    for (int c0 = 0; c0 < n; c0 += ctx->G) {
        int nc = n - c0 < ctx->G ? n - c0 : ctx->G;
        const void *d;
        RET(in_ptr(ctx, src, (size_t)c0 * N, (size_t)nc * N, loc, &d));
// ... 122 lines not shown
        if (accum) {
            int *tmp_acc = (int *)((char *)ctx->scratch + lines_bytes);
            k_accum_untranspose<<<dim3(64, nc), 256, 0, ctx->stream>>>(ctx->accum, tmp_acc, na, nr, ctx->acc_cap);
            KCHK("k_accum_untranspose");
            RET(out_copy(ctx, accum, (size_t)c0 * acc_n * 4, tmp_acc, (size_t)nc * acc_n * 4, loc));
        }
        if (lines_dev) {
            Span sp(ctx, KID_SORT);
            k_hough_sort<<<dim3(1, nc), 1024, 0, ctx->stream>>>(ctx->peaks, ctx->counters, lines_dev, max_lines, nr, (float)rho,
                                                               (float)theta, ctx->peak_cap);
            KCHK("k_hough_sort");
        }
        HIPCHK(hipMemcpyAsync(cnt.data(), ctx->counters, (size_t)nc * C_COUNT * sizeof(int), hipMemcpyDeviceToHost, ctx->stream));
        RET(sync(ctx, nc));
        for (int i = 0; i < nc; i++) {
            if (cnt[(size_t)i * C_COUNT + C_OVERFLOW]) {
                lfdmi_ctx *sp = get_spill(ctx);
                if (!sp) return fail(ctx, LFDMI_ERR_CAPACITY, "Hough lists too small for this image");
                int rc = hough_api(sp, img + (size_t)(c0 + i) * N, 1, h, w, rho, theta, threshold, max_lines,
                                   lines ? lines + (size_t)(c0 + i) * max_lines * 2 : nullptr, n_lines ? n_lines + c0 + i : nullptr,
                                   accum ? accum + (size_t)(c0 + i) * acc_n : nullptr, loc);
                if (rc) { ctx->err = sp->err; return rc; }
                ctx->n_spilled++;
                continue;
            }
            int total = cnt[(size_t)i * C_COUNT + C_NPEAK_EQU];
            if (n_lines) {
                if (loc == LFDMI_DEVICE) HIPCHK(hipMemcpy(n_lines + c0 + i, &total, 4, hipMemcpyHostToDevice));
                else n_lines[c0 + i] = total;
            }
            if (lines_dev) {
                int m = total < max_lines ? total : max_lines;
                if (m > 0)
                    HIPCHK(hipMemcpy((char *)lines + (size_t)(c0 + i) * max_lines * 8, lines_dev + (size_t)i * max_lines * 2, (size_t)m * 8,
                                     loc == LFDMI_DEVICE ? hipMemcpyDeviceToDevice : hipMemcpyDeviceToHost));
            }
        }
    }
    return 0;
}

extern "C" int lfdmi_hough_lines(lfdmi_ctx *ctx, const uint8_t *img, int n, int h, int w, double rho, double theta, int threshold,
                                 int max_lines, float *lines, int32_t *n_lines, int loc) {
    return hough_api(ctx, img, n, h, w, rho, theta, threshold, max_lines, lines, n_lines, nullptr, loc);
}
extern "C" int lfdmi_hough_accum(lfdmi_ctx *ctx, const uint8_t *img, int n, int h, int w, double rho, double theta, int32_t *accum, int loc) {
    return hough_api(ctx, img, n, h, w, rho, theta, 1, 0, nullptr, nullptr, accum, loc);
}

static int stage_catalog(lfdmi_ctx *ctx, const lfdmi_catalog *cat, int f0, int nc, lfdmi_catalog *dev) {
    size_t m = (size_t)cat->max_obj;
    *dev = *cat;
    if (cat->loc == LFDMI_DEVICE) {
        dev->count = cat->count + f0;
        dev->rowc = cat->rowc + f0 * m * 5; dev->colc = cat->colc + f0 * m * 5;
        dev->psfmag = cat->psfmag + f0 * m * 5; dev->petro90 = cat->petro90 + f0 * m * 5;
        dev->nobserve = cat->nobserve + f0 * m; dev->ndetect = cat->ndetect + f0 * m;
        return 0;
    }
    size_t b5 = (size_t)nc * m * 5 * 4, b1 = (size_t)nc * m * 4, bc = (size_t)nc * 4;
    size_t total = 4 * b5 + 2 * b1 + bc + 256;
    if (ctx->cat_bytes < total) {
        if (ctx->cat_dev) { HIPCHK(hipStreamSynchronize(ctx->stream)); HIPCHK(hipFree(ctx->cat_dev)); ctx->cat_dev = nullptr; ctx->cat_bytes = 0; }
        HIPCHK(hipMalloc(&ctx->cat_dev, total));
        ctx->cat_bytes = total;
    }
    char *p = (char *)ctx->cat_dev;
    auto up = [&](const void *src, size_t off_elems_bytes, size_t bytes, const void **out) -> int {
        HIPCHK(hipMemcpyAsync(p, (const char *)src + off_elems_bytes, bytes, hipMemcpyHostToDevice, ctx->stream));
        *out = p;
        p += (bytes + 15) & ~(size_t)15;
        return 0;
    };
    RET(up(cat->count, (size_t)f0 * 4, bc, (const void **)&dev->count));
    RET(up(cat->rowc, f0 * m * 20, b5, (const void **)&dev->rowc));
    RET(up(cat->colc, f0 * m * 20, b5, (const void **)&dev->colc));
    RET(up(cat->psfmag, f0 * m * 20, b5, (const void **)&dev->psfmag));
    RET(up(cat->petro90, f0 * m * 20, b5, (const void **)&dev->petro90));
    RET(up(cat->nobserve, f0 * m * 4, b1, (const void **)&dev->nobserve));
    RET(up(cat->ndetect, f0 * m * 4, b1, (const void **)&dev->ndetect));
    return 0;
}

static int run_removestars(lfdmi_ctx *ctx, float *frames_dev, int f0, int nc, int h, int w, const lfdmi_catalog *cat,
                           const lfdmi_rs_params *rs, bool fill = true) {
    if (!cat || cat->max_obj <= 0) return 0;
    if (!rs || rs->filter_index < 0 || rs->filter_index > 4) return fail(ctx, LFDMI_ERR_ARG, "removestars params");
    lfdmi_catalog dev;
    RET(stage_catalog(ctx, cat, f0, nc, &dev));
    RsDev p;
    p.defaultxy = rs->defaultxy; p.maxxy = rs->maxxy; p.magcount = rs->magcount; p.filter_index = rs->filter_index;
    p.pixscale = rs->pixscale; p.maxmagdiff = rs->maxmagdiff; p.filter_cap = rs->filter_cap;
    size_t need = (size_t)nc * cat->max_obj;
    if (ctx->rs_boxes_cap < need) {
        if (ctx->rs_boxes) { HIPCHK(hipStreamSynchronize(ctx->stream)); HIPCHK(hipFree(ctx->rs_boxes)); ctx->rs_boxes = nullptr; ctx->rs_boxes_cap = 0; }
        if (ctx->rs_sboxes) { HIPCHK(hipFree(ctx->rs_sboxes)); ctx->rs_sboxes = nullptr; }
        HIPCHK(hipMalloc(&ctx->rs_boxes, need * sizeof(int4)));
        ctx->rs_boxes_cap = need;
    }
    ctx->rs_sorted = cat->max_obj > ctx->rs_sort_min && h < RS_SORT_MAXH && (w % 32) == 0 && w <= RS_MAXW;
    if (ctx->rs_sorted) {
        if (!ctx->rs_sboxes) HIPCHK(hipMalloc(&ctx->rs_sboxes, ctx->rs_boxes_cap * sizeof(int4)));
        const size_t nrs = (size_t)nc * (h + 1);
        if (ctx->rs_rowstart_cap < nrs) {
            if (ctx->rs_rowstart) { HIPCHK(hipStreamSynchronize(ctx->stream)); HIPCHK(hipFree(ctx->rs_rowstart)); ctx->rs_rowstart = nullptr; }
            HIPCHK(hipMalloc(&ctx->rs_rowstart, nrs * sizeof(int)));
            ctx->rs_rowstart_cap = nrs;
        }
        ctx->rs_hmax = 2 * std::max(rs->maxxy, rs->defaultxy);
    }
    int4 *boxes = ctx->rs_boxes;
    {
        Span sp(ctx, KID_REMOVESTARS);
        k_rs_boxes<<<dim3((cat->max_obj + 255) / 256, nc), 256, 0, ctx->stream>>>(h, w, cat->max_obj, dev.count, dev.rowc, dev.colc, dev.psfmag,
                                                                               dev.petro90, dev.nobserve, dev.ndetect, p, boxes);
        KCHK("k_rs_boxes");
        ctx->rs_count_dev = dev.count;
        ctx->rs_max_obj = cat->max_obj;
        if (ctx->rs_sorted) {
            k_rs_sort<<<nc, 1024, 0, ctx->stream>>>(h, cat->max_obj, dev.count, boxes, ctx->rs_sboxes, ctx->rs_rowstart);
            KCHK("k_rs_sort");
        }
        if (fill) {
            if (ctx->rs_sorted)
                k_rs_fill_bands<<<dim3((h + RS_BAND_ROWS - 1) / RS_BAND_ROWS, nc), 256, 0, ctx->stream>>>(frames_dev, h, w, cat->max_obj, ctx->rs_sboxes,
                                                                                                     ctx->rs_rowstart, ctx->rs_hmax);
            else
                k_rs_fill<<<dim3((cat->max_obj + 3) / 4, nc), 256, 0, ctx->stream>>>(frames_dev, h, w, cat->max_obj, dev.count, boxes, 0);
            KCHK("k_rs_fill");
        }
    }
    return 0;
}

static void bind_thread(const std::vector<int> &cpus);
static void blot_host_frames(float *frames, int nc, int h, int w, const lfdmi_catalog *cat, int f0, const int4 *boxes,
                             const std::vector<int> &cpus) {
    size_t N = (size_t)h * w;
    auto work = [&](int a, int b) {
        bind_thread(cpus);
        for (int f = a; f < b; f++) {
            int n_obj = cat->count[f0 + f];
            float *img = frames + (size_t)f * N;
            for (int i = 0; i < n_obj && i < cat->max_obj; i++) {
                int4 bx = boxes[(size_t)f * cat->max_obj + i];
                if (bx.y <= bx.x || bx.w <= bx.z) continue;
                for (int r = bx.x; r < bx.y; r++) memset(img + (size_t)r * w + bx.z, 0, (size_t)(bx.w - bx.z) * sizeof(float));
            }
        }
    };
    int nt = nc >= 32 ? 8 : (nc >= 8 ? 4 : 1);
    if (nt == 1) { work(0, nc); return; }
    std::vector<std::thread> th;
    for (int t = 0; t < nt; t++) th.emplace_back(work, nc * t / nt, nc * (t + 1) / nt);
    for (auto &x : th) x.join();
}

extern "C" int lfdmi_remove_stars(lfdmi_ctx *ctx, float *img, int n, int h, int w, const lfdmi_catalog *cat,
                                  const lfdmi_rs_params *rs, int loc) {
    RET(check_shape(ctx, n, h, w));
    if (!img || !cat) return fail(ctx, LFDMI_ERR_ARG, "NULL argument");
    size_t N = (size_t)h * w;
    for (int c0 = 0; c0 < n; c0 += ctx->G) {
        int nc = n - c0 < ctx->G ? n - c0 : ctx->G;
        const void *d;
        RET(in_ptr(ctx, img, (size_t)c0 * N * 4, (size_t)nc * N * 4, loc, &d));
        RET(run_removestars(ctx, (float *)d, c0, nc, h, w, cat, rs));
        if (loc == LFDMI_HOST) RET(out_copy(ctx, img, (size_t)c0 * N * 4, d, (size_t)nc * N * 4, loc));
        RET(sync(ctx, nc));
    }
    return 0;
}

#define GENERAL_QUIET_CHUNKS 8
static bool general_again(lfdmi_ctx *c, bool on, const int *flags, int n) {
    bool need = false;
    for (int i = 0; i < n; i++) need = need || (flags[i] & PASS_FLAG_GENERAL);
    if (on) {
        c->n_general_chunks++;
        if (need) c->quiet_chunks = 0;
        else if (c->frame_ccl && ++c->quiet_chunks >= GENERAL_QUIET_CHUNKS) { c->general_seen = false; c->quiet_chunks = 0; }
        return false;
    }
    if (!need) return false;
    c->general_seen = true;
    c->general_on = true;
    c->quiet_chunks = 0;
    c->n_general_reruns++;
    return true;
}

static CallChunk chunk_start(lfdmi_ctx *ctx, int c0, int nc) {
    ctx->general_on = !ctx->frame_ccl || ctx->general_seen;
    return CallChunk{c0, nc, ctx->general_on, ctx->scan_fused, ctx->n_cap_growths};
}

static bool chunk_again(lfdmi_ctx *ctx, const CallChunk &ch, const int *flags, const lfdmi_result *rec, size_t rstride, int n_scales,
                        bool may_grow) {
    if (scan_gave_up(ctx, flags, ch.nc, ch.scan_fused)) return true;
    bool over = false;
    for (int s = 0; s < n_scales; s++)
        for (int i = 0; i < ch.nc; i++) over = over || rec[s * rstride + i].status == LFDMI_ERR_CAPACITY;
    if (over && (ctx->n_cap_growths > ch.growths || (may_grow && grow_caps(ctx, rec, ch.nc, rstride, n_scales)))) return true;
    return general_again(ctx, ch.general_on, flags, ch.nc);
}

static int enqueue_pass_chunk(lfdmi_ctx *ctx, const void *d, int dtype, int nc, int h, int w, int flip, int prep_mode, bool dim,
                              const lfdmi_params *p, int n_scales, const double *rhos, lfdmi_result *rec_h, size_t hstride, int *flags_h,
                              float *hl) {
    const size_t G = (size_t)ctx->G;
    for (int s = 0; s < n_scales; s++) {
        k_init_results<<<(nc + 63) / 64, 64, 0, ctx->stream>>>(ctx->res_dev + s * G, ctx->pass_flags, nc);
        KCHK("k_init_results");
    }
    RET(run_front(ctx, d, dtype, nc, h, w, flip, prep_mode, dim, p, nullptr));
    for (int s = 0; s < n_scales; s++) {
        RET(run_tail(ctx, nc, h, w, rhos[s], dim, p, nullptr, nullptr, ctx->res_dev + s * G, s > 0));
        HIPCHK(hipMemcpyAsync(rec_h + s * hstride, ctx->res_dev + s * G, (size_t)nc * sizeof(lfdmi_result), hipMemcpyDeviceToHost, ctx->stream));
    }
    if (hl) HIPCHK(hipMemcpyAsync(hl, ctx->lines, (size_t)nc * 2 * p->nlinesInSet * 2 * sizeof(float), hipMemcpyDeviceToHost, ctx->stream));
    HIPCHK(hipMemcpyAsync(flags_h, ctx->pass_flags, (size_t)nc * sizeof(int), hipMemcpyDeviceToHost, ctx->stream));
    return 0;
}

static int pass_api(lfdmi_ctx *ctx, const void *img, int dtype, int n, int h, int w, int flip, int prep_mode, bool dim,
                    const lfdmi_params *p, int n_scales, const double *rhos, lfdmi_result *results, size_t rstride, float *lines_equ,
                    float *lines_box, int loc);

static int finish_pass_frames(lfdmi_ctx *ctx, const void *img, int dtype, int c0, int nc, int h, int w, int flip, int prep_mode, bool dim,
                              const lfdmi_params *p, int n_scales, const double *rhos, lfdmi_result *host, size_t hstride, const float *hl,
                              lfdmi_result *results, size_t rstride, float *lines_equ, float *lines_box, int loc) {
    const size_t N = (size_t)h * w, es = dtype_size(dtype);
    const int K = p->nlinesInSet;
    for (int i = 0; i < nc; i++) {
        bool spill = false;
        for (int s = 0; s < n_scales; s++) spill = spill || host[s * hstride + i].status == LFDMI_ERR_CAPACITY;
        if (spill) {
            lfdmi_ctx *sp = get_spill(ctx);
            if (sp) {
                lfdmi_result one[LFDMI_MAX_SCALES];
                int rc = pass_api(sp, (const char *)img + (size_t)(c0 + i) * N * es, dtype, 1, h, w, flip, prep_mode, dim, p, n_scales, rhos,
                                  one, 1, lines_equ ? lines_equ + (size_t)(c0 + i) * 2 * K : nullptr,
                                  lines_box ? lines_box + (size_t)(c0 + i) * 2 * K : nullptr, loc);
                if (rc) { ctx->err = sp->err; return rc; }
                for (int s = 0; s < n_scales; s++) results[s * rstride + c0 + i] = one[s];
                ctx->n_spilled++;
                continue;
            }
        }
        for (int s = 0; s < n_scales; s++) {
            dictify(h, w, &host[s * hstride + i]);
            results[s * rstride + c0 + i] = host[s * hstride + i];
        }
        const lfdmi_result &last = host[(size_t)(n_scales - 1) * hstride + i];
        bool have = last.detection && last.status == 0;
        for (int s = 0; s < 2; s++) {
            float *dst = s ? lines_box : lines_equ;
            if (!dst) continue;
            for (int k = 0; k < 2 * K; k++) dst[(size_t)(c0 + i) * 2 * K + k] = have ? hl[((size_t)i * 2 + s) * 2 * K + k] : 0.f;
        }
    }
    return 0;
}

static int pass_prologue(lfdmi_ctx *ctx, const void *img, int dtype, int n, int h, int w, bool dim, const lfdmi_params *p, int n_scales,
                         const double *rhos, const lfdmi_result *results, lfdmi_ctx **ws) {
    RET(check_shape(ctx, n, h, w));
    RET(check_params(ctx, p, dim));
    if (!img || !results || dtype < 0 || dtype > 2) return fail(ctx, LFDMI_ERR_ARG, "bad argument");
    if (n_scales < 1 || n_scales > LFDMI_MAX_SCALES) return fail(ctx, LFDMI_ERR_ARG, "n_scales out of range");
    if (dtype == LFDMI_U8 && dim) return fail(ctx, LFDMI_ERR_DTYPE, "dim pass needs a float image (numpy refuses uint8 += float)");
    RET(call_workspace(ctx, h, w, rhos ? rhos : &p->houghMethod, n_scales, LFD_PI / 180, ws));
    if (*ws == ctx) ctx->keep_equ = ctx->stages_valid = ctx->stage_mode != 0;
    return 0;
}

static int pass_api(lfdmi_ctx *ctx, const void *img, int dtype, int n, int h, int w, int flip, int prep_mode, bool dim,
                    const lfdmi_params *p, int n_scales, const double *rhos, lfdmi_result *results, size_t rstride, float *lines_equ,
                    float *lines_box, int loc) {
    lfdmi_ctx *ws;
    RET(pass_prologue(ctx, img, dtype, n, h, w, dim, p, n_scales, rhos, results, &ws));
    if (!rhos) rhos = &p->houghMethod;
    if (ws != ctx) {
        int rc = pass_api(ws, img, dtype, n, h, w, flip, prep_mode, dim, p, n_scales, rhos, results, rstride, lines_equ, lines_box, loc);
        if (rc) ctx->err = ws->err;
        return rc;
    }
    size_t N = (size_t)h * w, es = dtype_size(dtype);
    int K = p->nlinesInSet;
    const size_t G = (size_t)ctx->G;
    std::vector<lfdmi_result> host(G * n_scales);
    std::vector<float> hl(G * 2 * K * 2);
    std::vector<int> flags(G);
// ... 181 lines not shown
                            fs->err = e;
                            fs->stop = true;
                            published = true;
                            break;
                        }
                        next_issue++;
                    }
                    if (published) fs->cv.notify_all();
                }
            }
        };
        std::vector<std::thread> th;
        for (int t = 1; t < T; t++) th.emplace_back(worker, t);
        worker(0);
        for (auto &x : th) x.join();
    });
}

static double feed_now() {
    timespec ts;
    clock_gettime(CLOCK_MONOTONIC, &ts);
    return ts.tv_sec * 1e3 + ts.tv_nsec * 1e-6;
}
static int feed_wait(lfdmi_ctx *ctx, FeedState *fs, int j) {
    {
        std::unique_lock<std::mutex> lk(fs->mu);
        fs->cv.wait(lk, [&] { return fs->issued > j || fs->stop; });
        if (fs->issued <= j) {
            const hipError_t e = fs->err;
            return fail(ctx, LFDMI_ERR_HIP, std::string("host-frame feed: ") + (e != hipSuccess ? hipGetErrorString(e) : "stopped"));
        }
    }
    HIPCHK(hipStreamWaitEvent(ctx->stream, ctx->feed_up[j & 1], 0));
    return 0;
}
static void feed_done(FeedState *fs, int chunks_done) {
    std::lock_guard<std::mutex> lk(fs->mu);
    fs->done = chunks_done;
    fs->cv.notify_all();
}

__global__ void __launch_bounds__(256) k_bswap32(uint4 *p, size_t n16) {
    for (size_t k = (size_t)blockIdx.x * 256 + threadIdx.x; k < n16; k += (size_t)gridDim.x * 256) {
        uint4 v = p[k];
        v.x = __builtin_bswap32(v.x); v.y = __builtin_bswap32(v.y); v.z = __builtin_bswap32(v.z); v.w = __builtin_bswap32(v.w);
        p[k] = v;
    }
}
static int run_bswap(lfdmi_ctx *ctx, void *dev, size_t bytes) {
    Span sp(ctx, KID_MISC);
    const size_t n16 = bytes / 16;
    if (n16) {
        k_bswap32<<<(unsigned)std::min<size_t>((n16 + 255) / 256, 16384), 256, 0, ctx->stream>>>((uint4 *)dev, n16);
        KCHK("k_bswap32");
    }
    if (bytes % 16) {
        std::vector<uint32_t> tail((bytes % 16) / 4);
        char *q = (char *)dev + n16 * 16;
        HIPCHK(hipMemcpyAsync(tail.data(), q, tail.size() * 4, hipMemcpyDeviceToHost, ctx->stream));
        HIPCHK(hipStreamSynchronize(ctx->stream));
        for (auto &v : tail) v = __builtin_bswap32(v);
        HIPCHK(hipMemcpyAsync(q, tail.data(), tail.size() * 4, hipMemcpyHostToDevice, ctx->stream));
        HIPCHK(hipStreamSynchronize(ctx->stream));
    }
    return 0;
}

static int pinned_upload(lfdmi_ctx *ctx, const char *src, size_t bytes, int kc) {
    char *dst = (char *)ctx->feed_dev[kc & 1];
    hipStream_t copy = ctx->feed_copy, copy2 = ctx->feed_streams == 2 ? ctx->feed_copy2 : ctx->feed_copy;
    int k = 0;
    for (size_t o = 0; o < bytes; o += FEED_PIECE, k++)
        HIPCHK(hipMemcpyAsync(dst + o, src + o, std::min<size_t>(FEED_PIECE, bytes - o), hipMemcpyHostToDevice, (k & 1) ? copy2 : copy));
    if (copy2 != copy) {
        HIPCHK(hipEventRecord(ctx->feed_mid, copy2));
        HIPCHK(hipStreamWaitEvent(copy, ctx->feed_mid, 0));
    }
    HIPCHK(hipEventRecord(ctx->feed_up[kc & 1], copy));
    return 0;
}

static int enqueue_detect_passes(lfdmi_ctx *ctx, const void *d, int nc, int h, int w, const lfdmi_params *bright, const lfdmi_params *dim,
                                 bool dual, bool delta) {
    k_init_results<<<(nc + 63) / 64, 64, 0, ctx->stream>>>(ctx->res_dev, ctx->pass_flags, nc);
    KCHK("k_init_results");
    struct DualState { lfdmi_ctx *c; ~DualState() { c->dual_state = 0; } } dual_guard{ctx};
    struct DeltaState { lfdmi_ctx *c; ~DeltaState() { c->delta_state = 0; } } delta_guard{ctx};
    ctx->cur_pass = 0;
    ctx->dual_state = 0;
    ctx->delta_state = delta ? 1 : 0;
    RET(run_pass(ctx, d, LFDMI_F32, nc, h, w, 1, LFDMI_PREP_BRIGHT, false, bright, nullptr, ctx->need_dim, (dual || delta) ? dim : nullptr));
    ctx->cur_pass = 1;
    ctx->dual_state = dual ? 2 : 0;
    ctx->delta_state = delta ? 2 : 0;
    RET(run_pass(ctx, d, LFDMI_F32, nc, h, w, 1, LFDMI_PREP_BRIGHT_THEN_DIM, true, dim, ctx->need_dim, nullptr));
    ctx->cur_pass = 0;
    ctx->dual_state = 0;
    ctx->delta_state = 0;
    RET(rs_fill_point(ctx, -1));
    if (ctx->rs_fill_inflight) { HIPCHK(hipStreamWaitEvent(ctx->stream, ctx->ev_rsfill, 0)); ctx->rs_fill_inflight = false; }
    return 0;
}

static int detect_impl(lfdmi_ctx *ctx, void *frames_v, int dtype, int n, int h, int w, const lfdmi_catalog *cat,
                       const lfdmi_rs_params *rs, const lfdmi_params *bright, const lfdmi_params *dim,
                       lfdmi_result *results, int loc, int cat_f0 = 0);

static int finish_detect_frames(lfdmi_ctx *ctx, float *frames, int dtype, int c0, int nc, int h, int w, const lfdmi_catalog *cat,
                                const lfdmi_rs_params *rs, const lfdmi_params *bright, const lfdmi_params *dim, lfdmi_result *host,
                                lfdmi_result *results, int loc, int cat_f0, std::thread *blotter) {
    const size_t N = (size_t)h * w;
    const bool be = dtype == LFDMI_F32_BE;
    for (int i = 0; i < nc; i++) {
        if (host[i].status == LFDMI_ERR_CAPACITY) {
            lfdmi_ctx *sp = get_spill(ctx);
            if (sp) {
                if (blotter && blotter->joinable()) blotter->join();
                int rc = detect_impl(sp, frames + (size_t)(c0 + i) * N, dtype, 1, h, w, be ? cat : nullptr, be ? rs : nullptr, bright, dim,
                                     &results[c0 + i], loc == LFDMI_HOST_PINNED ? LFDMI_HOST : loc, cat_f0 + c0 + i);
                if (rc) { ctx->err = sp->err; return rc; }
                ctx->n_spilled++;
                continue;
            }
        }
        dictify(h, w, &host[i]);
        results[c0 + i] = host[i];
    }
    return 0;
}

static int feed_chunk_frames(const lfdmi_ctx *ctx, int n, size_t N, bool pinned) {
    size_t fpc = (ctx->feed_chunk_bytes ? ctx->feed_chunk_bytes : (size_t)(800u << 20)) / (N * 4);
    int per = (int)std::min<size_t>((size_t)ctx->G, std::max<size_t>(1, fpc));
    if (pinned) {
        const char *pe = getenv("LFDMI_PINNED_CHUNKS");
        const int pin_div = pe ? std::max(1, atoi(pe)) : 1;
        per = std::max(std::min(per, 8), std::min(per, (n + pin_div - 1) / pin_div));
    }
    return per;
}

static void dim_front_end(lfdmi_ctx *ctx, int w, const lfdmi_params *dim, bool *dual_out, bool *delta_out) {
    const bool dual = ctx->fuse_dual && can_fuse_prep_erode(ctx, LFDMI_F32, w, dim->erodeKernel, dim->erode_kh, dim->erode_kw);
    const bool delta = !dual && ctx->delta_dim && (w % 32) == 0 && (float)dim->addFlux >= 0.0f && (float)dim->addFlux <= 0.999f &&
                       (float)dim->minFlux <= 0.5f &&
                       dim->erode_kh * dim->erode_kw <= 25 &&
                       can_fuse_prep_erode(ctx, LFDMI_F32, w, dim->erodeKernel, dim->erode_kh, dim->erode_kw);
    *dual_out = dual;
    *delta_out = delta;
}

struct FoldState {
    lfdmi_ctx *c;
    ~FoldState() {
        if (c->rs_fill_inflight) { (void)hipStreamSynchronize(c->side[0]); (void)hipStreamSynchronize(c->side[1]); c->rs_fill_inflight = false; }
        c->rs_fold = false; c->rs_fill_frames = nullptr; c->rs_fill_part = 0;
    }
};

static int detect_prologue(lfdmi_ctx *ctx, const char *fn, void *frames, int *dtype, int n, int h, int w, const lfdmi_catalog *cat,
                           const lfdmi_rs_params *rs, const lfdmi_params *bright, const lfdmi_params *dim, const lfdmi_result *results,
                           int loc, lfdmi_ctx **ws, bool *dual, bool *delta) {
    RET(check_shape(ctx, n, h, w));
    RET(check_params(ctx, bright, false));
    RET(check_params(ctx, dim, true));
    if (!frames || !results) return fail(ctx, LFDMI_ERR_ARG, "NULL argument");
    if (*dtype != LFDMI_F32 && *dtype != LFDMI_F32_BE) return fail(ctx, LFDMI_ERR_DTYPE, std::string(fn) + ": frames must be LFDMI_F32 or LFDMI_F32_BE");
    if (loc != LFDMI_HOST && loc != LFDMI_DEVICE && loc != LFDMI_HOST_PINNED) return fail(ctx, LFDMI_ERR_ARG, "bad loc");
    if (cat && cat->max_obj > 0 && (!rs || rs->filter_index < 0 || rs->filter_index > 4)) return fail(ctx, LFDMI_ERR_ARG, "removestars params");
    const double rhos[2] = {bright->houghMethod, dim->houghMethod};
    RET(call_workspace(ctx, h, w, rhos, 2, LFD_PI / 180, ws));
    if (*ws != ctx) return 0;
    if (*dtype == LFDMI_F32_BE && loc == LFDMI_DEVICE) {
        RET(run_bswap(ctx, frames, (size_t)n * h * w * 4));
        *dtype = LFDMI_F32;
    }
    ctx->keep_equ = ctx->stages_valid = ctx->stage_mode == 1;
    dim_front_end(ctx, w, dim, dual, delta);
    return 0;
}

static bool blot_on_host(const lfdmi_catalog *cat, bool on_host, int dtype) {
    return cat && on_host && cat->loc == LFDMI_HOST && dtype != LFDMI_F32_BE;
}

static int enqueue_detect_front(lfdmi_ctx *ctx, float *frames, const void *d, int dtype, bool on_host, int c0, int nc, int h, int w,
                                const lfdmi_catalog *cat, const lfdmi_rs_params *rs, int cat_f0, bool delta, int4 *squares) {
    const size_t N = (size_t)h * w;
    const bool be = dtype == LFDMI_F32_BE, host_blot = blot_on_host(cat, on_host, dtype);
    if (be) RET(run_bswap(ctx, (void *)d, (size_t)nc * N * 4));
    const bool copy_back = cat && on_host && !host_blot && !be;
    ctx->rs_fold = cat && cat->max_obj > 0 && ctx->rs_fold_on && delta && w <= RS_MAXW && !copy_back;
    ctx->rs_fill_frames = nullptr;
    if (!cat) return 0;
    RET(run_removestars(ctx, (float *)d, cat_f0 + c0, nc, h, w, cat, rs, !ctx->rs_fold));
    if (ctx->rs_fold && !on_host) { ctx->rs_fill_frames = (float *)d; ctx->rs_fill_part = 0; ctx->rs_fill_nc = nc; ctx->rs_fill_h = h; ctx->rs_fill_w = w; }
    if (copy_back) RET(out_copy(ctx, frames, (size_t)c0 * N * 4, d, (size_t)nc * N * 4, LFDMI_HOST));
    if (host_blot && cat->max_obj > 0)
        HIPCHK(hipMemcpyAsync(squares, ctx->rs_boxes, (size_t)nc * cat->max_obj * sizeof(int4), hipMemcpyDeviceToHost, ctx->stream));
    return 0;
}

static int detect_impl(lfdmi_ctx *ctx, void *frames_v, int dtype, int n, int h, int w, const lfdmi_catalog *cat,
                       const lfdmi_rs_params *rs, const lfdmi_params *bright, const lfdmi_params *dim,
                       lfdmi_result *results, int loc, int cat_f0) {
    float *frames = (float *)frames_v;
    lfdmi_ctx *ws;
    bool dual, delta;
    RET(detect_prologue(ctx, "lfdmi_detect_batch_raw", frames, &dtype, n, h, w, cat, rs, bright, dim, results, loc, &ws, &dual, &delta));
    if (ws != ctx) {
        int rc = detect_impl(ws, frames, dtype, n, h, w, cat, rs, bright, dim, results, loc, cat_f0);
        if (rc) ctx->err = ws->err;
        return rc;
    }
    const bool pinned = loc == LFDMI_HOST_PINNED, on_host = loc != LFDMI_DEVICE;
    const bool host_blot = blot_on_host(cat, on_host, dtype);
    size_t N = (size_t)h * w;
    int *const flags = (int *)ctx->res_host;
    lfdmi_result *const host = (lfdmi_result *)((char *)ctx->res_host + (size_t)ctx->G * sizeof(int));
    std::vector<int4> boxes;
    int per = ctx->G;
    const bool feed = loc == LFDMI_HOST && ctx->feed_chunk_bytes > 0 && (size_t)n * N * 4 >= (64u << 20);
    if (feed || pinned) {
        per = feed_chunk_frames(ctx, n, N, pinned);
        RET(feed_prepare(ctx, (size_t)std::min(per, n) * N * 4, feed));
    }
    FeedState fs;
    std::thread blotter;
    struct FeedJoin {
        lfdmi_ctx *c; FeedState *f; std::thread *b; bool feed;
        ~FeedJoin() {
            { std::lock_guard<std::mutex> lk(f->mu); f->stop = true; f->cv.notify_all(); }
            if (f->th.joinable()) f->th.join();
            if (feed) { (void)hipStreamSynchronize(c->feed_copy); (void)hipStreamSynchronize(c->feed_copy2); }
            if (b->joinable()) b->join();
        }
    } feed_join{ctx, &fs, &blotter, feed || pinned};
    if (feed) feed_start(ctx, &fs, (const char *)frames, N * 4, n, per);
    if (pinned && n > 0) RET(pinned_upload(ctx, (const char *)frames, (size_t)std::min(per, n) * N * 4, 0));
    const int fail_chunk = ctx->fail_chunk;
    ctx->fail_chunk = -1;
    for (int c0 = 0, kc = 0; c0 < n; c0 += per, kc++) {
        int nc = n - c0 < per ? n - c0 : per;
        const void *d;
        if (kc == fail_chunk) return fail(ctx, LFDMI_ERR_ARG, "lfdmi_debug_fail_chunk: injected failure");
        if (feed) {
            d = ctx->feed_dev[kc & 1];
            RET(feed_wait(ctx, &fs, kc));
        } else if (pinned) {
            d = ctx->feed_dev[kc & 1];
            if (c0 + per < n)
                RET(pinned_upload(ctx, (const char *)frames + (size_t)(c0 + per) * N * 4, (size_t)std::min(per, n - c0 - per) * N * 4, kc + 1));
            HIPCHK(hipStreamWaitEvent(ctx->stream, ctx->feed_up[kc & 1], 0));
        } else RET(in_ptr(ctx, frames, (size_t)c0 * N * 4, (size_t)nc * N * 4, loc, &d));
        FoldState fold_guard{ctx};
        if (host_blot) boxes.resize((size_t)nc * std::max(0, cat->max_obj));
        RET(enqueue_detect_front(ctx, frames, d, dtype, on_host, c0, nc, h, w, cat, rs, cat_f0, delta, boxes.data()));
        if (host_blot) {
            double t0_ = feed && getenv("LFDMI_FEED_TRACE") ? feed_now() : 0;
            HIPCHK(hipStreamSynchronize(ctx->stream));
            if (t0_ > 0) fprintf(stderr, "[feed] chunk %d: upload + remove_stars synced after %.2f ms (t=%.2f)\n", kc, feed_now() - t0_, feed_now());
        }
        bool blotted = false;
        for (int grow_tries = 0;;) {
            const CallChunk ch = chunk_start(ctx, c0, nc);
            RET(enqueue_detect_passes(ctx, d, nc, h, w, bright, dim, dual, delta));
            if (host_blot && !blotted) {
                if (blotter.joinable()) blotter.join();
                blotter = std::thread([=, bx = boxes, cpus = ctx->feed_cpus] { blot_host_frames(frames + (size_t)c0 * N, nc, h, w, cat, cat_f0 + c0, bx.data(), cpus); });
                blotted = true;
            }
            HIPCHK(hipMemcpyAsync(ctx->res_host, ctx->pass_flags, (size_t)ctx->G * sizeof(int) + (size_t)nc * sizeof(lfdmi_result), hipMemcpyDeviceToHost, ctx->stream));
            double t0_ = feed && getenv("LFDMI_FEED_TRACE") ? feed_now() : 0;
            HIPCHK(hipStreamSynchronize(ctx->stream));
            if (t0_ > 0) fprintf(stderr, "[feed] chunk %d (%d frames): passes synced after %.2f ms (t=%.2f)\n", kc, nc, feed_now() - t0_, feed_now());
            if (!chunk_again(ctx, ch, flags, host, 1, 1, grow_tries < 4)) break;
            grow_tries += ctx->n_cap_growths > ch.growths;
        }
// ... 315 lines not shown
    RET(idle(ctx));
    HIPCHK(hipMemcpyAsync(dst, ctx->prof, (size_t)n * 16 * sizeof(long long), hipMemcpyDeviceToHost, ctx->stream));
    HIPCHK(hipStreamSynchronize(ctx->stream));
    return 0;
}

extern "C" int lfdmi_debug_tail(lfdmi_ctx *ctx, int n, int kmax, const float *h1, const int32_t *n1, const float *h2, const int32_t *n2,
                                int navg, double dro, double thetaTresh, double lineSetTresh, int which, int h, int w, lfdmi_result *out) {
    if (!ctx || n < 0 || !h1 || !h2 || !n1 || !n2 || !out || kmax < 1 || navg < 1 || navg > LFDMI_MAX_SET_LINES || (which != 1 && which != 2))
        return fail(ctx, LFDMI_ERR_ARG, "lfdmi_debug_tail: bad argument");
    RET(idle(ctx));
    HIPCHK(hipSetDevice(ctx->device));
    const int G = ctx->G, K = navg;
    std::vector<float> lines((size_t)G * 2 * K * 2);
    std::vector<int> cnt((size_t)G * C_COUNT);
    for (int c0 = 0; c0 < n; c0 += G) {
        const int nc = std::min(G, n - c0);
        std::fill(lines.begin(), lines.end(), 0.f);
        std::fill(cnt.begin(), cnt.end(), 0);
        for (int i = 0; i < nc; i++) {
            const int a = n1[c0 + i], b = n2[c0 + i];
            if (a < 0 || a > kmax || b < 0 || b > kmax) return fail(ctx, LFDMI_ERR_ARG, "lfdmi_debug_tail: line count");
            for (int k = 0; k < K && k < a; k++) { lines[((size_t)i * 2 + 0) * K * 2 + 2 * k] = h1[((size_t)(c0 + i) * kmax + k) * 2]; lines[((size_t)i * 2 + 0) * K * 2 + 2 * k + 1] = h1[((size_t)(c0 + i) * kmax + k) * 2 + 1]; }
            for (int k = 0; k < K && k < b; k++) { lines[((size_t)i * 2 + 1) * K * 2 + 2 * k] = h2[((size_t)(c0 + i) * kmax + k) * 2]; lines[((size_t)i * 2 + 1) * K * 2 + 2 * k + 1] = h2[((size_t)(c0 + i) * kmax + k) * 2 + 1]; }
            cnt[(size_t)i * C_COUNT + C_DETECT] = 1;
            cnt[(size_t)i * C_COUNT + C_NPEAK_EQU] = a;
            cnt[(size_t)i * C_COUNT + C_NPEAK_BOX] = b;
        }
        HIPCHK(hipMemcpyAsync(ctx->lines, lines.data(), (size_t)nc * 2 * K * 2 * sizeof(float), hipMemcpyHostToDevice, ctx->stream));
        HIPCHK(hipMemcpyAsync(ctx->counters, cnt.data(), (size_t)nc * C_COUNT * sizeof(int), hipMemcpyHostToDevice, ctx->stream));
        k_init_results<<<(nc + 63) / 64, 64, 0, ctx->stream>>>(ctx->res_dev, ctx->pass_flags, nc);
        KCHK("k_init_results");
        TailParams tp;
        tp.navg = navg; tp.dro = dro; tp.thetaTresh = thetaTresh; tp.lineSetTresh = lineSetTresh; tp.which = which;
        k_finalize<<<(nc + 63) / 64, 64, 0, ctx->stream>>>(ctx->lines, ctx->counters, ctx->res_dev, nullptr, ctx->pass_flags, nullptr, tp, nc);
        KCHK("k_finalize");
        HIPCHK(hipMemcpyAsync(out + c0, ctx->res_dev, (size_t)nc * sizeof(lfdmi_result), hipMemcpyDeviceToHost, ctx->stream));
        HIPCHK(hipStreamSynchronize(ctx->stream));
        for (int i = 0; i < nc; i++) dictify(h, w, &out[c0 + i]);
    }
    return 0;
}

extern "C" int lfdmi_debug_trig(lfdmi_ctx *ctx, int n, const double *y, const double *x, float *angle_deg, float *cos_half, float *sin_half) {
    if (!ctx || n < 0 || !y || !x || !angle_deg || !cos_half || !sin_half) return LFDMI_ERR_ARG;
    RET(idle(ctx));
    if (n == 0) return 0;
    HIPCHK(hipSetDevice(ctx->device));
    RET(ensure_scratch(ctx, (size_t)n * (2 * sizeof(double) + 3 * sizeof(float))));
    double *dy = (double *)ctx->scratch, *dx = dy + n;
    float *o = (float *)(dx + n);
    HIPCHK(hipMemcpyAsync(dy, y, (size_t)n * sizeof(double), hipMemcpyHostToDevice, ctx->stream));
    HIPCHK(hipMemcpyAsync(dx, x, (size_t)n * sizeof(double), hipMemcpyHostToDevice, ctx->stream));
    k_debug_trig<<<(n + 255) / 256, 256, 0, ctx->stream>>>(dy, dx, o, o + n, o + 2 * (size_t)n, n);
    KCHK("k_debug_trig");
    HIPCHK(hipMemcpyAsync(angle_deg, o, (size_t)n * sizeof(float), hipMemcpyDeviceToHost, ctx->stream));
    HIPCHK(hipMemcpyAsync(cos_half, o + n, (size_t)n * sizeof(float), hipMemcpyDeviceToHost, ctx->stream));
    HIPCHK(hipMemcpyAsync(sin_half, o + 2 * (size_t)n, (size_t)n * sizeof(float), hipMemcpyDeviceToHost, ctx->stream));
    HIPCHK(hipStreamSynchronize(ctx->stream));
    return 0;
}

extern "C" int lfdmi_set_stage_images(lfdmi_ctx *ctx, int mode) {
    if (!ctx || mode < -1 || mode > 1) return LFDMI_ERR_ARG;
    ctx->stage_mode = mode;
    return 0;
}

extern "C" int lfdmi_get_stage(lfdmi_ctx *ctx, int slot, int which, int h, int w, uint8_t *dst, int loc) {
    if (!ctx || !dst || slot < 0 || slot >= ctx->G) return LFDMI_ERR_ARG;
    RET(idle(ctx));
    if (ctx->last_h <= 0) return fail(ctx, LFDMI_ERR_ARG, "no call has run yet");
    if (h != ctx->last_h || w != ctx->last_w) return fail(ctx, LFDMI_ERR_ARG, "lfdmi_get_stage: the last call worked on a different shape");
    size_t N = (size_t)h * w, BW = (size_t)h * LFD_WQ(w);
    HIPCHK(hipSetDevice(ctx->device));
    const uint8_t *src = nullptr;
    if (which != LFDMI_STAGE_CANNY && which != LFDMI_STAGE_BOX && !ctx->stages_valid && !(which == LFDMI_STAGE_ERODED && ctx->eroded_valid))
        return fail(ctx, LFDMI_ERR_ARG, "lfdmi_get_stage: the last call did not keep the 8-bit stage images (lfdmi_set_stage_images)");
    if (which == LFDMI_STAGE_GRAY) src = ctx->gray + slot * N;
    else if (which == LFDMI_STAGE_EQU) src = ctx->equ + slot * N;
    else if (which == LFDMI_STAGE_EQUALIZED || which == LFDMI_STAGE_ERODED) {
        RET(ensure_scratch(ctx, N));
        const uint8_t *plane = (which == LFDMI_STAGE_EQUALIZED ? ctx->gray : ctx->tmp) + slot * N;
        k_apply_lut<<<dim3(512, 1), 256, 0, ctx->stream>>>(plane, ctx->lut + slot * 256, (uint8_t *)ctx->scratch, N);
        KCHK("k_apply_lut");
        src = (const uint8_t *)ctx->scratch;
    } else if (which == LFDMI_STAGE_CANNY || which == LFDMI_STAGE_BOX) {
        const u64 *bits = (which == LFDMI_STAGE_CANNY ? ctx->edgeb : ctx->boxb) + slot * BW;
        RET(ensure_scratch(ctx, N));
        RET(expand_bits(ctx, bits, (uint8_t *)ctx->scratch, 1, h, w));
        src = (const uint8_t *)ctx->scratch;
    } else return fail(ctx, LFDMI_ERR_ARG, "unknown stage");
    RET(out_copy(ctx, dst, 0, src, N, loc));
    return sync(ctx, 1);
}

LFD_HIDDEN int ctx_begin(lfdmi_ctx *ctx) {
    RET(idle(ctx));
    if (hipSetDevice(ctx->device) != hipSuccess) return fail(ctx, LFDMI_ERR_HIP, "hipSetDevice");
    (void)hipGetLastError();
    return 0;
}
LFD_HIDDEN int ctx_fail(lfdmi_ctx *ctx, int code, const std::string &msg) { return fail(ctx, code, msg); }
LFD_HIDDEN hipStream_t ctx_stream(lfdmi_ctx *ctx) { return ctx->stream; }
LFD_HIDDEN int ctx_device(lfdmi_ctx *ctx) { return ctx->device; }
LFD_HIDDEN void **ctx_defocus(lfdmi_ctx *ctx, void (*release)(lfdmi_ctx *)) {
    if (release) ctx->defocus_free = release;
    return &ctx->defocus;
}

extern "C" void lfdmi_default_trail_params(lfdmi_trail_params *o) {
    if (!o) return;
    o->half_width = 32; o->seg_len = 64; o->n_iter = 3; o->wing = 8;
    o->k_sig = 5.0; o->prof_half = 24.0; o->prof_step = 0.1; o->pixscale = 0.396;
}

static int trail_buf(lfdmi_ctx *ctx, void **p, size_t *cap, size_t need) {
    if (*cap >= need) return 0;
    if (*p) { HIPCHK(hipStreamSynchronize(ctx->stream)); HIPCHK(hipFree(*p)); *p = nullptr; ctx->trail.bytes -= *cap; *cap = 0; }
    HIPCHK(hipMalloc(p, need));
    *cap = need;
    ctx->trail.bytes += need;
    return 0;
}

static void trail_blank(lfdmi_trail *o, int status) {
    const double nan = NAN;
    o->status = status; o->n_pos = 0; o->n_seg = 0; o->min_valid = 0;
    o->rho = o->theta = o->x1 = o->y1 = o->x2 = o->y2 = nan;
    o->background = o->noise = o->peak = o->fwhm = o->fwhm_arcsec = o->depth = nan;
}

#define TRAIL_CHUNK 64

extern "C" int lfdmi_measure_trails(lfdmi_ctx *ctx, const void *frames, int dtype, int n, int h, int w, int loc, const lfdmi_result *rec,
                                    const lfdmi_catalog *cat, const lfdmi_rs_params *rs, const lfdmi_trail_params *p_in, lfdmi_trail *out,
                                    float *profiles) {
    RET(check_shape(ctx, n, h, w));
    if (n > 0 && (!frames || !rec || !out)) return fail(ctx, LFDMI_ERR_ARG, "NULL argument");
    if (dtype != LFDMI_F32 && dtype != LFDMI_F32_BE) return fail(ctx, LFDMI_ERR_DTYPE, "lfdmi_measure_trails takes LFDMI_F32 / LFDMI_F32_BE frames");
    if (loc != LFDMI_HOST && loc != LFDMI_DEVICE && loc != LFDMI_HOST_PINNED) return fail(ctx, LFDMI_ERR_ARG, "bad loc");
    if (h < 2 || w < 2) return fail(ctx, LFDMI_ERR_ARG, "frame smaller than 2 x 2");
    lfdmi_trail_params q;
    if (p_in) q = *p_in; else lfdmi_default_trail_params(&q);
    const double kd = q.prof_half / q.prof_step;
    const int K = (std::isfinite(kd) && kd >= 1 && kd <= TRAIL_MAX_K) ? (int)llround(kd) : 0;
    if (q.half_width < 1 || q.half_width > TRAIL_MAX_R || q.seg_len < 2 || q.seg_len > 64 || q.n_iter < 0 || q.n_iter > 16 ||
        q.wing < 1 || q.wing > q.half_width || !std::isfinite(q.k_sig) || !std::isfinite(q.pixscale) || !(q.prof_step > 0) ||
        K == 0 || fabs((double)K * q.prof_step - q.prof_half) > 1e-9 * q.prof_half || q.wing > q.prof_half)
        return fail(ctx, LFDMI_ERR_ARG, "trail params out of range (include/lfdmi.h: lfdmi_trail_params)");
    const bool stars = cat && cat->max_obj > 0;
    if (stars && (!rs || rs->filter_index < 0 || rs->filter_index > 4)) return fail(ctx, LFDMI_ERR_ARG, "removestars params");
    const int nb = 2 * K + 1;
    const size_t N = (size_t)h * w;
    std::vector<int> act;
    for (int i = 0; i < n; i++) {
        if (rec[i].found) act.push_back(i);
        else trail_blank(&out[i], LFDMI_TRAIL_NOT_FOUND);
        if (profiles && !rec[i].found) for (int b = 0; b < nb; b++) profiles[(size_t)i * nb + b] = NAN;
    }
    const int nact = (int)act.size();
    if (nact == 0) return 0;

    TrailDev dp;
    dp.R = q.half_width; dp.L = q.seg_len; dp.n_iter = q.n_iter; dp.wing = q.wing; dp.K = K;
    dp.maxpos = (int)ceil(sqrt((double)ctx->H * ctx->H + (double)ctx->W * ctx->W)) + 2;
    dp.maxseg = dp.maxpos / dp.L + 1;
    dp.be = dtype == LFDMI_F32_BE; dp.h = h; dp.w = w; dp.wq = (w + 31) / 32;
    dp.k_sig = q.k_sig; dp.P = q.prof_half; dp.step = q.prof_step; dp.pixscale = q.pixscale;
    const int nu = 2 * dp.R + 1;
    const int CH = std::min(ctx->G, TRAIL_CHUNK);
    auto &T = ctx->trail;
    RET(trail_buf(ctx, &T.st, &T.st_c, (size_t)nact * sizeof(TrailState)));
    RET(trail_buf(ctx, &T.segm, &T.segm_c, (size_t)CH * dp.maxseg * nu * sizeof(float)));
    RET(trail_buf(ctx, &T.sA, &T.sA_c, (size_t)CH * dp.maxseg * sizeof(double)));
    RET(trail_buf(ctx, &T.sC, &T.sC_c, (size_t)CH * dp.maxseg * sizeof(double)));
    RET(trail_buf(ctx, &T.sSig, &T.sSig_c, (size_t)CH * dp.maxseg * sizeof(int)));
    RET(trail_buf(ctx, &T.prof, &T.prof_c, (size_t)nact * nb * sizeof(float)));
    RET(trail_buf(ctx, &T.cnt, &T.cnt_c, (size_t)CH * nb * sizeof(int)));
    RET(trail_buf(ctx, &T.rec, &T.rec_c, (size_t)nact * 10 * sizeof(double)));
    if (stars) {
        RET(trail_buf(ctx, &T.planes, &T.planes_c, (size_t)CH * ctx->H * ((ctx->W + 31) / 32) * sizeof(uint32_t)));
        RET(trail_buf(ctx, &T.boxes, &T.boxes_c, (size_t)CH * cat->max_obj * sizeof(int4)));
    }
    if (loc != LFDMI_DEVICE) RET(trail_buf(ctx, &T.stage, &T.stage_c, (size_t)CH * N * 4));

    std::vector<TrailState> hs(nact);
    std::vector<int> first(1, 0);
    for (int k = 0, c0 = 0; c0 < n; c0 += CH) {
        int slot = 0;
        for (; k < nact && act[k] < c0 + CH; k++, slot++) {
            const int i = act[k];
            TrailState &s = hs[k];
            memset(&s, 0, sizeof(s));
            const double th = (double)rec[i].theta, rho = (double)rec[i].rho, c = cos(th), sn = sin(th);
            s.fx = rho * c; s.fy = rho * sn; s.dx = -sn; s.dy = c;
            s.img = loc == LFDMI_DEVICE ? (const void *)((const char *)frames + (size_t)i * N * 4)
                                        : (const void *)((char *)T.stage + (size_t)slot * N * 4);
            s.frame = k; s.slot = slot; s.chunk_frame = i - c0;
        }
        first.push_back(k);
    }
    HIPCHK(hipMemcpyAsync(T.st, hs.data(), (size_t)nact * sizeof(TrailState), hipMemcpyHostToDevice, ctx->stream));
    TrailState *st = (TrailState *)T.st;
    const uint32_t *planes = stars ? (const uint32_t *)T.planes : nullptr;
    for (int ci = 0, c0 = 0; c0 < n; c0 += CH, ci++) {
        const int a0 = first[ci], na = first[ci + 1] - a0, nc = std::min(CH, n - c0);
        if (na == 0) continue;
        if (loc != LFDMI_DEVICE)
            for (int k = a0; k < a0 + na; k++)
                HIPCHK(hipMemcpyAsync((char *)T.stage + (size_t)(k - a0) * N * 4, (const char *)frames + (size_t)act[k] * N * 4, N * 4,
                                      hipMemcpyHostToDevice, ctx->stream));
        if (stars) {
            lfdmi_catalog dev;
            RET(stage_catalog(ctx, cat, c0, nc, &dev));
            RsDev rp;
            rp.defaultxy = rs->defaultxy; rp.maxxy = rs->maxxy; rp.magcount = rs->magcount; rp.filter_index = rs->filter_index;
            rp.pixscale = rs->pixscale; rp.maxmagdiff = rs->maxmagdiff; rp.filter_cap = rs->filter_cap;
            k_rs_boxes<<<dim3((cat->max_obj + 255) / 256, nc), 256, 0, ctx->stream>>>(h, w, cat->max_obj, dev.count, dev.rowc, dev.colc,
                                                                                   dev.psfmag, dev.petro90, dev.nobserve, dev.ndetect, rp,
                                                                                   (int4 *)T.boxes);
            KCHK("k_rs_boxes");
            HIPCHK(hipMemsetAsync(T.planes, 0, (size_t)na * h * dp.wq * sizeof(uint32_t), ctx->stream));
            k_trail_mask<<<dim3((cat->max_obj + 3) / 4, na), 256, 0, ctx->stream>>>(st + a0, na, cat->max_obj, (const int4 *)T.boxes,
                                                                                   (uint32_t *)T.planes, dp);
            KCHK("k_trail_mask");
        }
        k_trail_init<<<(na + 63) / 64, 64, 0, ctx->stream>>>(st + a0, na, dp);
        KCHK("k_trail_init");
        for (int it = 0; it <= dp.n_iter; it++) {
            k_trail_seg<<<dim3(dp.maxseg, na), TRAIL_SEG_THREADS, 0, ctx->stream>>>(st + a0, na, planes, (float *)T.segm, dp);
            KCHK("k_trail_seg");
            k_trail_fit<<<na, 64, 0, ctx->stream>>>(st + a0, na, (const float *)T.segm, (double *)T.sA, (double *)T.sC, (int *)T.sSig,
                                                    it == dp.n_iter, dp);
            KCHK("k_trail_fit");
        }
        k_trail_prof<<<dim3(nb, na), 256, (size_t)dp.maxpos * sizeof(uint32_t), ctx->stream>>>(st + a0, na, planes, (float *)T.prof,
                                                                                              (int *)T.cnt, dp);
        KCHK("k_trail_prof");
        k_trail_final<<<na, 64, 0, ctx->stream>>>(st + a0, na, (float *)T.prof, (const int *)T.cnt, (double *)T.rec, dp);
        KCHK("k_trail_final");
    }
    std::vector<float> hp((size_t)nact * nb);
    std::vector<double> hr((size_t)nact * 10);
    HIPCHK(hipMemcpyAsync(hs.data(), T.st, (size_t)nact * sizeof(TrailState), hipMemcpyDeviceToHost, ctx->stream));
    HIPCHK(hipMemcpyAsync(hp.data(), T.prof, hp.size() * sizeof(float), hipMemcpyDeviceToHost, ctx->stream));
    HIPCHK(hipMemcpyAsync(hr.data(), T.rec, hr.size() * sizeof(double), hipMemcpyDeviceToHost, ctx->stream));
    RET(sync(ctx));
    for (int k = 0; k < nact; k++) {
        const TrailState &s = hs[k];
        const int i = act[k];
        if (s.status < 0) return fail(ctx, s.status, "lfdmi_measure_trails: a line longer than the workspace's tables");
        lfdmi_trail *o = &out[i];
        if (s.status != 0 || !s.done) {
            trail_blank(o, s.status ? s.status : LFDMI_TRAIL_TOO_FAINT);
            if (profiles) for (int b = 0; b < nb; b++) profiles[(size_t)i * nb + b] = NAN;
            continue;
        }
        const double *r = &hr[(size_t)k * 10];
        o->status = LFDMI_TRAIL_OK;
        o->n_pos = std::min(s.s1 * dp.L + dp.L, s.npos) - s.s0 * dp.L;
        o->n_seg = s.s1 - s.s0 + 1;
        o->min_valid = s.min_valid;
        line_rho_theta(s.fx, s.fy, s.dx, s.dy, &o->rho, &o->theta);
        o->x1 = r[0]; o->y1 = r[1]; o->x2 = r[2]; o->y2 = r[3];
        o->background = r[4]; o->noise = r[5]; o->peak = r[6];
        o->fwhm = r[7]; o->fwhm_arcsec = r[8]; o->depth = r[9];
        if (profiles) memcpy(profiles + (size_t)i * nb, &hp[(size_t)k * nb], nb * sizeof(float));
    }
    return 0;
}
```

Baseline: 63970.

## Fold per-step init, LUT pair, and finalize-next into fewer kernel launches

Replaces the separate init-results kernel and several memsets with one per-frame init kernel, optionally folded into k_rs_boxes. It computes both bright and dim LUTs in one paired launch, and merges the bright-pass finalize with the counter reset and active-permutation build. The aim is to cut kernel-launch and memset overhead across the detect pipeline. The cost is a cross-stage 'done' bitmask whose state must stay correct across calls, plus a second LUT buffer.

```diff
diff --git a/lfd_amd/csrc/k_hough.h b/lfd_amd/csrc/k_hough.h
--- a/lfd_amd/csrc/k_hough.h
+++ b/lfd_amd/csrc/k_hough.h
@@ -434,11 +434,9 @@
     int which;
 };
 
-__global__ void k_finalize(const float *lines, const int *counters, lfdmi_result *res, int *need_dim,
-                           int *pass_flags, const int *active, TailParams tp, int G) {
-    int g = blockIdx.x * blockDim.x + threadIdx.x;
-    if (g >= G) return;
-    if (active && !active[g]) { if (need_dim) need_dim[g] = 0; return; }
+__device__ __forceinline__ int finalize_frame(const float *lines, const int *counters, lfdmi_result *res, int *need_dim,
+                                              int *pass_flags, const int *active, const TailParams &tp, int g) {
+    if (active && !active[g]) { if (need_dim) need_dim[g] = 0; return 0; }
     const int *cnt = counters + g * C_COUNT;
     lfdmi_result r = res[g];
     r.detection = cnt[C_DETECT];
@@ -492,7 +490,35 @@
     }
     res[g] = r;
     pass_flags[g] |= (tp.which == 1) ? (r.detection ? 1 : 0) : (2 | (r.detection ? 4 : 0));
-    if (need_dim) need_dim[g] = (r.found == 0 && r.status == 0) ? 1 : 0;
+    const int nd = (r.found == 0 && r.status == 0) ? 1 : 0;
+    if (need_dim) need_dim[g] = nd;
+    return nd;
+}
+
+__global__ void k_finalize(const float *lines, const int *counters, lfdmi_result *res, int *need_dim,
+                           int *pass_flags, const int *active, TailParams tp, int G) {
+    int g = blockIdx.x * blockDim.x + threadIdx.x;
+    if (g >= G) return;
+    finalize_frame(lines, counters, res, need_dim, pass_flags, active, tp, g);
+}
+
+__global__ void __launch_bounds__(1024)
+k_finalize_next(const float *lines, int *counters, lfdmi_result *res, int *need_dim, int *pass_flags, TailParams tp, int G, int *perm) {
+    __shared__ int act[1024];
+    const int t = threadIdx.x;
+    if (t < G) act[t] = finalize_frame(lines, counters, res, need_dim, pass_flags, nullptr, tp, t);
+    __syncthreads();
+    for (int k = t; k < G * C_COUNT; k += blockDim.x) counters[k] = 0;
+    if (t >= 64 || !perm) return;
+    int base = 0;
+    for (int pass = 0; pass < 2; pass++)
+        for (int i0 = 0; i0 < G; i0 += 64) {
+            const int i = i0 + t;
+            const bool on = i < G && ((act[i] != 0) == (pass == 0));
+            const u64 bal = __ballot(on);
+            if (on) perm[base + __popcll(bal & ((1ull << t) - 1ull))] = i;
+            base += __popcll(bal);
+        }
 }
 
 __global__ void k_hough_reset(int *counters, int G) {
@@ -502,6 +528,36 @@
     cnt[C_NPIX_EQU] = 0; cnt[C_NPIX_BOX] = 0; cnt[C_NPIXB_EQU] = 0; cnt[C_NPIXB_BOX] = 0; cnt[C_NPEAK_EQU] = 0; cnt[C_NPEAK_BOX] = 0;
     cnt[C_NNZ_EQU] = 0; cnt[C_NNZ_BOX] = 0;
 }
+
+struct StepInit {
+    lfdmi_result *res;
+    size_t res_stride;
+    int n_scales;
+    int *pass_flags, *counters, *hist, *hist2;
+    u64 *cellbm, *cellbm2;
+    int bm_words;
+};
+__device__ __forceinline__ void step_init_frame(const StepInit &s, int g) {
+    const int t = threadIdx.x, nt = blockDim.x;
+    if (t < s.n_scales) {
+        lfdmi_result r;
+        r.status = 0; r.found = 0; r.rho = 0.f; r.theta = 0.f;
+        r.x1 = r.y1 = r.x2 = r.y2 = 0;
+        r.n_lines_equ = r.n_lines_box = 0; r.detection = 0; r.rejected_by_theta = 0;
+        s.res[(size_t)t * s.res_stride + g] = r;
+    }
+    if (t == 0) s.pass_flags[g] = 0;
+    if (t < C_COUNT) s.counters[g * C_COUNT + t] = 0;
+    for (int k = t; k < 256; k += nt) {
+        s.hist[g * 256 + k] = 0;
+        if (s.hist2) s.hist2[g * 256 + k] = 0;
+    }
+    for (int k = t; k < s.bm_words; k += nt) {
+        s.cellbm[(size_t)g * s.bm_words + k] = 0;
+        if (s.cellbm2) s.cellbm2[(size_t)g * s.bm_words + k] = 0;
+    }
+}
+__global__ void __launch_bounds__(256) k_step_init(StepInit s) { step_init_frame(s, blockIdx.x); }
 
 __global__ void k_init_results(lfdmi_result *res, int *pass_flags, int G) {
     int g = blockIdx.x * blockDim.x + threadIdx.x;
diff --git a/lfd_amd/csrc/k_image.h b/lfd_amd/csrc/k_image.h
--- a/lfd_amd/csrc/k_image.h
+++ b/lfd_amd/csrc/k_image.h
@@ -16,8 +16,9 @@
 
 __global__ void __launch_bounds__(256)
 k_rs_boxes(int h, int w, int max_obj, const int *count, const float *rowc, const float *colc, const float *psfmag,
-           const float *petro90, const int *nobserve, const int *ndetect, RsDev p, int4 *boxes) {
+           const float *petro90, const int *nobserve, const int *ndetect, RsDev p, int4 *boxes, StepInit init) {
     const int f = blockIdx.y, i = blockIdx.x * 256 + threadIdx.x;
+    if (init.res && blockIdx.x == 0) step_init_frame(init, f);
     if (i >= max_obj) return;
     int r0 = 0, r1 = 0, c0 = 0, c1 = 0;
     if (i < count[f]) {
@@ -670,10 +671,8 @@
     if (sh[threadIdx.x]) atomicAdd(&hist[g * 256 + threadIdx.x], sh[threadIdx.x]);
 }
 
-__global__ void __launch_bounds__(256)
-k_lut(const int *hist, int total, uint8_t *lut, const int *active) {
-    int g = blockIdx.x, t = threadIdx.x;
-    if (active && !active[g]) return;
+__device__ __forceinline__ void lut_frame(const int *hist, int total, uint8_t *lut, int g) {
+    const int t = threadIdx.x;
     __shared__ int cum[256];
     __shared__ int first;
     int hv = hist[g * 256 + t];
@@ -698,6 +697,16 @@
         out = sat_u8_f32(__fmul_rn((float)(cum[t] - cum[f]), scale));
     }
     lut[g * 256 + t] = (uint8_t)out;
+}
+__global__ void __launch_bounds__(256)
+k_lut(const int *hist, int total, uint8_t *lut, const int *active) {
+    const int g = blockIdx.x;
+    if (active && !active[g]) return;
+    lut_frame(hist, total, lut, g);
+}
+__global__ void __launch_bounds__(256)
+k_lut_pair(const int *hist, const int *hist2, int total, uint8_t *lut, uint8_t *lut2) {
+    lut_frame(blockIdx.y ? hist2 : hist, total, blockIdx.y ? lut2 : lut, blockIdx.x);
 }
 
 __global__ void __launch_bounds__(256)
diff --git a/lfd_amd/csrc/lfdmi.hip b/lfd_amd/csrc/lfdmi.hip
--- a/lfd_amd/csrc/lfdmi.hip
+++ b/lfd_amd/csrc/lfdmi.hip
@@ -126,6 +126,13 @@
     int *perm = nullptr;
     const int *perm_cur = nullptr;
     bool use_perm = true;
+    bool fold_init = true;
+    bool fold_lut = true;
+    bool fold_next = true;
+    uint8_t *lut2 = nullptr;
+    const uint8_t *lut_last = nullptr;
+    enum { DONE_INIT = 1, DONE_ZERO = 2, DONE_ZERO2 = 4, DONE_LUT2 = 8, DONE_NEXT = 16 };
+    int done = 0;
     int *perm_tiles = nullptr;
     bool use_tile_perm = true;
     bool sky_fast = true;
@@ -410,6 +417,7 @@
     RET(dmalloc(ctx, &ctx->tmp, G * N));
     RET(dmalloc(ctx, &ctx->equ, G * N));
     RET(dmalloc(ctx, &ctx->lut, G * 256));
+    RET(dmalloc(ctx, &ctx->lut2, G * 256));
     RET(dmalloc(ctx, &ctx->mask, (size_t)LFDMI_MAX_MORPH_K * LFDMI_MAX_MORPH_K * 2));
     RET(dmalloc(ctx, &ctx->candb, G * BW));
     RET(dmalloc(ctx, &ctx->strongb, G * BW));
@@ -448,6 +456,9 @@
     if (const char *e = getenv("LFDMI_RS_FILL_AT")) ctx->rs_fill_at = atoi(e);
     if (const char *e = getenv("LFDMI_RS_FILL_AT0")) ctx->rs_fill_at0 = atoi(e);
     if (const char *e = getenv("LFDMI_PERM")) ctx->use_perm = atoi(e) != 0;
+    if (const char *e = getenv("LFDMI_FOLD_INIT")) ctx->fold_init = atoi(e) != 0;
+    if (const char *e = getenv("LFDMI_FOLD_LUT")) ctx->fold_lut = atoi(e) != 0;
+    if (const char *e = getenv("LFDMI_FOLD_NEXT")) ctx->fold_next = atoi(e) != 0;
     RET(dmalloc(ctx, &ctx->fb_fg, G));
     RET(dmalloc(ctx, &ctx->fg_keys, G));
     HIPCHK(hipMemsetAsync(ctx->fg_keys, 0, G * sizeof(int), ctx->stream));
@@ -868,6 +879,12 @@
         KCHK("k_prep_hist");
     }
     Span sp(ctx, KID_LUT);
+    if (delta_dim && ctx->fold_lut && !active) {
+        k_lut_pair<<<dim3(nc, 2), 256, 0, ctx->stream>>>(ctx->hist, ctx->hist2, h * w, ctx->lut, ctx->lut2);
+        KCHK("k_lut_pair");
+        ctx->done |= lfdmi_ctx::DONE_LUT2;
+        return 0;
+    }
     k_lut<<<nc, 256, 0, ctx->stream>>>(ctx->hist, h * w, ctx->lut, active);
     KCHK("k_lut");
     return 0;
@@ -1455,7 +1472,7 @@
     int kh = dimp->erode_kh, kw = dimp->erode_kw;
     int BR = prep_erode_rows(ctx, w, kh);
     size_t lds = (size_t)(2 * BR + kh - 1) * (w + 32) + 16;
-    HIPCHK(hipMemsetAsync(ctx->zero_block2, 0, ctx->zero_bytes2, ctx->stream));
+    if (!(ctx->done & lfdmi_ctx::DONE_ZERO2)) HIPCHK(hipMemsetAsync(ctx->zero_block2, 0, ctx->zero_bytes2, ctx->stream));
     {
         Span sp(ctx, KID_PREP_DUAL);
         k_prep_erode<true, LFDMI_PREP_BRIGHT_THEN_DIM><<<dim3((h + BR - 1) / BR, nc), PE_THREADS, lds, ctx->stream>>>((const float *)src, h, w, flip, LFDMI_PREP_BRIGHT_THEN_DIM,
@@ -1464,6 +1481,12 @@
         KCHK("k_prep_dual");
     }
     Span sp(ctx, KID_LUT);
+    if (ctx->fold_lut) {
+        k_lut_pair<<<dim3(nc, 2), 256, 0, ctx->stream>>>(ctx->hist, ctx->hist2, h * w, ctx->lut, ctx->lut2);
+        KCHK("k_lut_pair");
+        ctx->done |= lfdmi_ctx::DONE_LUT2;
+        return 0;
+    }
     k_lut<<<nc, 256, 0, ctx->stream>>>(ctx->hist, h * w, ctx->lut, nullptr);
     KCHK("k_lut");
     return 0;
@@ -1472,18 +1495,25 @@
 static int run_front(lfdmi_ctx *ctx, const void *src, int dtype, int nc, int h, int w, int flip, int prep_mode, bool dim,
                      const lfdmi_params *p, const int *active, const lfdmi_params *dual_dim = nullptr) {
     const uint8_t *dil_src = ctx->gray;
+    const uint8_t *lut = ctx->lut;
     const u64 *bm = ctx->cellbm;
     ctx->eroded_valid = dim;
     ctx->perm_cur = nullptr;
+    const bool have_next = dim && (ctx->done & lfdmi_ctx::DONE_NEXT), have_lut2 = dim && (ctx->done & lfdmi_ctx::DONE_LUT2);
     if (active && ctx->use_perm) {
-        k_active_perm<<<1, 64, 0, ctx->stream>>>(active, nc, ctx->perm);
-        KCHK("k_active_perm");
+        if (!have_next) {
+            k_active_perm<<<1, 64, 0, ctx->stream>>>(active, nc, ctx->perm);
+            KCHK("k_active_perm");
+        }
         ctx->perm_cur = ctx->perm;
     }
     if (dim && ctx->delta_state == 2) {
-        HIPCHK(hipMemsetAsync(ctx->zero_block + ctx->zero_counters_off, 0, ctx->zero_bytes - ctx->zero_counters_off, ctx->stream));
-        HIPCHK(hipMemsetAsync(ctx->cellbm2, 0, (size_t)nc * ctx->bm_bands * CELLBM_WORDS * sizeof(u64), ctx->stream));
-        { Span sp(ctx, KID_LUT);
+        if (!have_next)
+            HIPCHK(hipMemsetAsync(ctx->zero_block + ctx->zero_counters_off, 0, ctx->zero_bytes - ctx->zero_counters_off, ctx->stream));
+        if (!(ctx->done & lfdmi_ctx::DONE_ZERO2))
+            HIPCHK(hipMemsetAsync(ctx->cellbm2, 0, (size_t)nc * ctx->bm_bands * CELLBM_WORDS * sizeof(u64), ctx->stream));
+        if (have_lut2) lut = ctx->lut2;
+        else { Span sp(ctx, KID_LUT);
           k_lut<<<nc, 256, 0, ctx->stream>>>(ctx->hist2, h * w, ctx->lut, active);
           KCHK("k_lut"); }
         RET(run_prep_erode(ctx, nullptr, nc, h, w, 0, 0, 0, 0, p->erode_kh, p->erode_kw, active, true));
@@ -1491,14 +1521,19 @@
         bm = ctx->cellbm2;
     } else
     if (dim && ctx->dual_state == 2) {
-        HIPCHK(hipMemsetAsync(ctx->zero_block + ctx->zero_counters_off, 0, ctx->zero_bytes - ctx->zero_counters_off, ctx->stream));
-        Span sp(ctx, KID_LUT);
-        k_lut<<<nc, 256, 0, ctx->stream>>>(ctx->hist2, h * w, ctx->lut, active);
-        KCHK("k_lut");
+        if (!have_next)
+            HIPCHK(hipMemsetAsync(ctx->zero_block + ctx->zero_counters_off, 0, ctx->zero_bytes - ctx->zero_counters_off, ctx->stream));
+        if (have_lut2) lut = ctx->lut2;
+        else {
+            Span sp(ctx, KID_LUT);
+            k_lut<<<nc, 256, 0, ctx->stream>>>(ctx->hist2, h * w, ctx->lut, active);
+            KCHK("k_lut");
+        }
         dil_src = ctx->tmp;
         bm = ctx->cellbm2;
     } else {
-    HIPCHK(hipMemsetAsync(ctx->zero_block, 0, ctx->zero_bytes, ctx->stream));
+    const bool zeroed = !dim && (ctx->done & lfdmi_ctx::DONE_ZERO), zeroed2 = !dim && (ctx->done & lfdmi_ctx::DONE_ZERO2);
+    if (!zeroed) HIPCHK(hipMemsetAsync(ctx->zero_block, 0, ctx->zero_bytes, ctx->stream));
     if (!dim && dual_dim && ctx->delta_state != 1) {
         RET(run_prep_dual(ctx, src, nc, h, w, flip, dual_dim));
     } else
@@ -1509,7 +1544,7 @@
         const bool wide = dim && p->erode_kw >= 7 && dtype == LFDMI_F32 && (w & 3) == 0 && p->erode_kh <= 33;
         if (dim) HIPCHK(hipMemsetAsync(ctx->zero_block2, 0, ctx->zero_bytes2, ctx->stream));
         const lfdmi_params *dd = (!dim && ctx->delta_state == 1) ? dual_dim : nullptr;
-        if (dd) HIPCHK(hipMemsetAsync(ctx->hist2, 0, (size_t)nc * 256 * sizeof(int), ctx->stream));
+        if (dd && !zeroed2) HIPCHK(hipMemsetAsync(ctx->hist2, 0, (size_t)nc * 256 * sizeof(int), ctx->stream));
         RET(run_prep(ctx, src, dtype, nc, h, w, flip, prep_mode, p->minFlux, p->addFlux, active, true, wide ? ctx->fullbits : nullptr, dd));
         RET(rs_fill_point(ctx, 1));
         if (dim) {
@@ -1525,24 +1560,25 @@
         }
     }
     }
+    ctx->lut_last = lut;
     if (p->gaussKernel > 0) {
-        RET(run_morph(ctx, dil_src, ctx->equ, ctx->equb, ctx->lut, p->dilateKernel, p->dilate_kh, p->dilate_kw, 0, nc, h, w, active));
+        RET(run_morph(ctx, dil_src, ctx->equ, ctx->equb, lut, p->dilateKernel, p->dilate_kh, p->dilate_kw, 0, nc, h, w, active));
         RET(ensure_scratch(ctx, (size_t)ctx->G * ctx->N));
         RET(run_gauss(ctx, ctx->equ, (uint8_t *)ctx->scratch, nc, h, w, p->gaussKernel, p->gaussSigma, active));
         RET(run_canny(ctx, (const uint8_t *)ctx->scratch, nc, h, w, 0, 255, active, false, true));
     } else if (can_fuse_dilate_canny(p->dilateKernel, p->dilate_kh, p->dilate_kw, w)) {
-        RET(run_dilate_canny(ctx, dil_src, nc, h, w, ctx->lut, p->dilate_kh, p->dilate_kw, active, ctx->use_cellbm ? bm : nullptr));
+        RET(run_dilate_canny(ctx, dil_src, nc, h, w, lut, p->dilate_kh, p->dilate_kw, active, ctx->use_cellbm ? bm : nullptr));
         RET(rs_fill_point(ctx, 2 + 10 * ctx->cur_pass));
         RET(run_canny(ctx, ctx->equ, nc, h, w, 0, 255, active, true, true));
     } else {
-        RET(run_morph(ctx, dil_src, ctx->equ, ctx->equb, ctx->lut, p->dilateKernel, p->dilate_kh, p->dilate_kw, 0, nc, h, w, active));
+        RET(run_morph(ctx, dil_src, ctx->equ, ctx->equb, lut, p->dilateKernel, p->dilate_kh, p->dilate_kw, 0, nc, h, w, active));
         RET(run_canny(ctx, ctx->equ, nc, h, w, 0, 255, active, false, true));
     }
     return run_rects(ctx, nc, h, w, p->contoursMode, p->contoursMethod, p->minAreaRectMinLen, p->lwTresh, active);
 }
 
 static int run_tail(lfdmi_ctx *ctx, int nc, int h, int w, double rho, bool dim, const lfdmi_params *p, const int *active,
-                    int *need_dim, lfdmi_result *res, bool again) {
+                    int *need_dim, lfdmi_result *res, bool again, bool then_dim = false) {
     if (again) {
         k_hough_reset<<<(nc + 63) / 64, 64, 0, ctx->stream>>>(ctx->counters, nc);
         KCHK("k_hough_reset");
@@ -1552,16 +1588,23 @@
     tp.navg = p->nlinesInSet; tp.dro = p->dro; tp.thetaTresh = p->thetaTresh; tp.lineSetTresh = p->lineSetTresh;
     tp.which = dim ? 2 : 1;
     Span sp(ctx, KID_FINALIZE);
+    if (then_dim && ctx->fold_next && !active && need_dim && nc <= 1024) {
+        k_finalize_next<<<1, (nc + 63) / 64 * 64, 0, ctx->stream>>>(ctx->lines, ctx->counters, res, need_dim, ctx->pass_flags, tp, nc,
+                                                                   ctx->use_perm ? ctx->perm : nullptr);
+        KCHK("k_finalize_next");
+        ctx->done |= lfdmi_ctx::DONE_NEXT;
+        return 0;
+    }
     k_finalize<<<(nc + 63) / 64, 64, 0, ctx->stream>>>(ctx->lines, ctx->counters, res, need_dim, ctx->pass_flags, active, tp, nc);
     KCHK("k_finalize");
     return 0;
 }
 
 static int run_pass(lfdmi_ctx *ctx, const void *src, int dtype, int nc, int h, int w, int flip, int prep_mode, bool dim,
-                    const lfdmi_params *p, const int *active, int *need_dim, const lfdmi_params *dual_dim = nullptr) {
+                    const lfdmi_params *p, const int *active, int *need_dim, const lfdmi_params *dual_dim = nullptr, bool then_dim = false) {
     RET(run_front(ctx, src, dtype, nc, h, w, flip, prep_mode, dim, p, active, dual_dim));
     ctx->perm_cur = nullptr;
-    return run_tail(ctx, nc, h, w, p->houghMethod, dim, p, active, need_dim, ctx->res_dev, false);
+    return run_tail(ctx, nc, h, w, p->houghMethod, dim, p, active, need_dim, ctx->res_dev, false, then_dim);
 }
 
 static void dictify(int h, int w, lfdmi_result *r) {
@@ -1850,8 +1893,24 @@
     return 0;
 }
 
+static StepInit step_init(lfdmi_ctx *ctx, int n_scales, bool both) {
+    StepInit s;
+    s.res = ctx->res_dev; s.res_stride = (size_t)ctx->G; s.n_scales = n_scales;
+    s.pass_flags = ctx->pass_flags; s.counters = ctx->counters; s.hist = ctx->hist; s.hist2 = both ? ctx->hist2 : nullptr;
+    s.cellbm = ctx->cellbm; s.cellbm2 = both ? ctx->cellbm2 : nullptr;
+    s.bm_words = ctx->bm_bands * CELLBM_WORDS;
+    return s;
+}
+static int run_step_init(lfdmi_ctx *ctx, int nc, int n_scales, bool both) {
+    k_step_init<<<nc, 256, 0, ctx->stream>>>(step_init(ctx, n_scales, both));
+    KCHK("k_step_init");
+    ctx->done |= lfdmi_ctx::DONE_INIT | lfdmi_ctx::DONE_ZERO | (both ? lfdmi_ctx::DONE_ZERO2 : 0);
+    return 0;
+}
+struct DoneState { lfdmi_ctx *c; ~DoneState() { c->done = 0; } };
+
 static int run_removestars(lfdmi_ctx *ctx, float *frames_dev, int f0, int nc, int h, int w, const lfdmi_catalog *cat,
-                           const lfdmi_rs_params *rs, bool fill = true) {
+                           const lfdmi_rs_params *rs, bool fill = true, bool init = false) {
     if (!cat || cat->max_obj <= 0) return 0;
     if (!rs || rs->filter_index < 0 || rs->filter_index > 4) return fail(ctx, LFDMI_ERR_ARG, "removestars params");
     lfdmi_catalog dev;
@@ -1880,9 +1939,12 @@
     int4 *boxes = ctx->rs_boxes;
     {
         Span sp(ctx, KID_REMOVESTARS);
+        StepInit si = step_init(ctx, 1, true);
+        if (!init) si.res = nullptr;
         k_rs_boxes<<<dim3((cat->max_obj + 255) / 256, nc), 256, 0, ctx->stream>>>(h, w, cat->max_obj, dev.count, dev.rowc, dev.colc, dev.psfmag,
-                                                                               dev.petro90, dev.nobserve, dev.ndetect, p, boxes);
+                                                                               dev.petro90, dev.nobserve, dev.ndetect, p, boxes, si);
         KCHK("k_rs_boxes");
+        if (init) ctx->done |= lfdmi_ctx::DONE_INIT | lfdmi_ctx::DONE_ZERO | lfdmi_ctx::DONE_ZERO2;
         ctx->rs_count_dev = dev.count;
         ctx->rs_max_obj = cat->max_obj;
         if (ctx->rs_sorted) {
@@ -1977,6 +2039,10 @@
                               const lfdmi_params *p, int n_scales, const double *rhos, lfdmi_result *rec_h, size_t hstride, int *flags_h,
                               float *hl) {
     const size_t G = (size_t)ctx->G;
+    DoneState done_guard{ctx};
+    ctx->done = 0;
+    if (ctx->fold_init) RET(run_step_init(ctx, nc, n_scales, false));
+    else
     for (int s = 0; s < n_scales; s++) {
         k_init_results<<<(nc + 63) / 64, 64, 0, ctx->stream>>>(ctx->res_dev + s * G, ctx->pass_flags, nc);
         KCHK("k_init_results");
@@ -2324,14 +2390,21 @@
 
 static int enqueue_detect_passes(lfdmi_ctx *ctx, const void *d, int nc, int h, int w, const lfdmi_params *bright, const lfdmi_params *dim,
                                  bool dual, bool delta) {
-    k_init_results<<<(nc + 63) / 64, 64, 0, ctx->stream>>>(ctx->res_dev, ctx->pass_flags, nc);
-    KCHK("k_init_results");
+    DoneState done_guard{ctx};
+    if (!(ctx->done & lfdmi_ctx::DONE_INIT)) {
+        ctx->done = 0;
+        if (ctx->fold_init) RET(run_step_init(ctx, nc, 1, true));
+        else {
+            k_init_results<<<(nc + 63) / 64, 64, 0, ctx->stream>>>(ctx->res_dev, ctx->pass_flags, nc);
+            KCHK("k_init_results");
+        }
+    }
     struct DualState { lfdmi_ctx *c; ~DualState() { c->dual_state = 0; } } dual_guard{ctx};
     struct DeltaState { lfdmi_ctx *c; ~DeltaState() { c->delta_state = 0; } } delta_guard{ctx};
     ctx->cur_pass = 0;
     ctx->dual_state = 0;
     ctx->delta_state = delta ? 1 : 0;
-    RET(run_pass(ctx, d, LFDMI_F32, nc, h, w, 1, LFDMI_PREP_BRIGHT, false, bright, nullptr, ctx->need_dim, (dual || delta) ? dim : nullptr));
+    RET(run_pass(ctx, d, LFDMI_F32, nc, h, w, 1, LFDMI_PREP_BRIGHT, false, bright, nullptr, ctx->need_dim, (dual || delta) ? dim : nullptr, true));
     ctx->cur_pass = 1;
     ctx->dual_state = dual ? 2 : 0;
     ctx->delta_state = delta ? 2 : 0;
@@ -2396,7 +2469,7 @@
     lfdmi_ctx *c;
     ~FoldState() {
         if (c->rs_fill_inflight) { (void)hipStreamSynchronize(c->side[0]); (void)hipStreamSynchronize(c->side[1]); c->rs_fill_inflight = false; }
-        c->rs_fold = false; c->rs_fill_frames = nullptr; c->rs_fill_part = 0;
+        c->rs_fold = false; c->rs_fill_frames = nullptr; c->rs_fill_part = 0; c->done = 0;
     }
 };
 
@@ -2435,7 +2508,8 @@
     ctx->rs_fold = cat && cat->max_obj > 0 && ctx->rs_fold_on && delta && w <= RS_MAXW && !copy_back;
     ctx->rs_fill_frames = nullptr;
     if (!cat) return 0;
-    RET(run_removestars(ctx, (float *)d, cat_f0 + c0, nc, h, w, cat, rs, !ctx->rs_fold));
+    ctx->done = 0;
+    RET(run_removestars(ctx, (float *)d, cat_f0 + c0, nc, h, w, cat, rs, !ctx->rs_fold, ctx->fold_init));
     if (ctx->rs_fold && !on_host) { ctx->rs_fill_frames = (float *)d; ctx->rs_fill_part = 0; ctx->rs_fill_nc = nc; ctx->rs_fill_h = h; ctx->rs_fill_w = w; }
     if (copy_back) RET(out_copy(ctx, frames, (size_t)c0 * N * 4, d, (size_t)nc * N * 4, LFDMI_HOST));
     if (host_blot && cat->max_obj > 0)
@@ -2917,7 +2991,7 @@
     else if (which == LFDMI_STAGE_EQUALIZED || which == LFDMI_STAGE_ERODED) {
         RET(ensure_scratch(ctx, N));
         const uint8_t *plane = (which == LFDMI_STAGE_EQUALIZED ? ctx->gray : ctx->tmp) + slot * N;
-        k_apply_lut<<<dim3(512, 1), 256, 0, ctx->stream>>>(plane, ctx->lut + slot * 256, (uint8_t *)ctx->scratch, N);
+        k_apply_lut<<<dim3(512, 1), 256, 0, ctx->stream>>>(plane, (ctx->lut_last ? ctx->lut_last : ctx->lut) + slot * 256, (uint8_t *)ctx->scratch, N);
         KCHK("k_apply_lut");
         src = (const uint8_t *)ctx->scratch;
     } else if (which == LFDMI_STAGE_CANNY || which == LFDMI_STAGE_BOX) {
@@ -3054,7 +3128,7 @@
             rp.pixscale = rs->pixscale; rp.maxmagdiff = rs->maxmagdiff; rp.filter_cap = rs->filter_cap;
             k_rs_boxes<<<dim3((cat->max_obj + 255) / 256, nc), 256, 0, ctx->stream>>>(h, w, cat->max_obj, dev.count, dev.rowc, dev.colc,
                                                                                    dev.psfmag, dev.petro90, dev.nobserve, dev.ndetect, rp,
-                                                                                   (int4 *)T.boxes);
+                                                                                   (int4 *)T.boxes, StepInit{});
             KCHK("k_rs_boxes");
             HIPCHK(hipMemsetAsync(T.planes, 0, (size_t)na * h * dp.wq * sizeof(uint32_t), ctx->stream));
             k_trail_mask<<<dim3((cat->max_obj + 3) / 4, na), 256, 0, ctx->stream>>>(st + a0, na, cat->max_obj, (const int4 *)T.boxes,
```

Result: no change. 64150, median of 6 (+0.3%).
